# jackvial/tuatara

Hardware: AMD Instinct MI355X
Metric: pages/sec whole-node (1024x768, ~40 crops/page) (higher is better)
Workload: dtype f16x4

## Files before the change

include/tuatara_hip_debug.h:

```cpp
#ifndef TUATARA_HIP_DEBUG_H
#define TUATARA_HIP_DEBUG_H

#include "tuatara_hip.h"

#ifdef __cplusplus
extern "C" {
#endif

int ttr_dbg_conv(ttr_engine* e, const float* in0, int C0, const float* in1, int C1, int relu0, int relu1, int B, int H, int W,
                 int ks, int dil, const float* wgt, const float* bias, int Cout, int act, float* out);

int ttr_dbg_split_gemm(ttr_engine* e, const float* x, int M, int K, const float* w, const float* bias, int N, int np, int act, int out_planes,
                       const float* resid, int cfg, float* out);
int ttr_dbg_conv_pool(ttr_engine* e, const float* in0, int C0, int B, int H, int W, int ks, const float* wgt, const float* bias,
                      int Cout, int act, int pool_relu, float* out_full, float* out_pool);
int ttr_dbg_craft_taps(ttr_engine* e, const uint8_t* canvas, int B, int H, int W, float* heat_out);
int ttr_dbg_craft_tap_count(ttr_engine* e);
int ttr_dbg_craft_tap_info(ttr_engine* e, int i, char* text, size_t cap, int dims[7]);
int ttr_dbg_craft_tap_read(ttr_engine* e, int i, float* out);
void ttr_set_gemm_config(int cfg);
void ttr_set_decoder_mode(int mode);
int ttr_set_tuning(const char* key, int value);
void ttr_last_host_us(ttr_engine* e, float out[8]);
int ttr_dbg_attn_enc(ttr_engine* e, const float* qkv, int N, float* out);
int ttr_dbg_cross_attn(ttr_engine* e, const float* q, const float* kvmem, int N, int R, float* out);
int ttr_dbg_qkv_attn(ttr_engine* e, const float* x, int N, const float* w, const float* b, float* out);
int ttr_dbg_mlp(ttr_engine* e, const float* x, int M, const float* ln_g, const float* ln_b, float eps, const float* w1, const float* b1, const float* w2,
                const float* b2, const float* nln_g, const float* nln_b, float* x_out, float* nln_out, const float* att, const float* wp, const float* bp);
int ttr_dbg_dec_stamps(unsigned long long* out);
int ttr_dbg_dec_stamps_ext(unsigned long long* out, int n);
int ttr_bench_conv(ttr_engine* e, int B, int H, int W, int C0, int C1, int ks, int dil, int Cout, int act, int f32_resid,
                   int iters, float* avg_us);

int ttr_dbg_min_area_rect(const float* xy, int n, float* rect5);
int ttr_dbg_tcp_share(int rank, int world, const char* addr, int port, void* buf, size_t bytes);
int ttr_dbg_component_rect(int area, int x0, int y0, int x1, int y1, const int32_t* rows, int H, int W, float* rect5);
int ttr_dbg_box_geometry(const float* rect5, float ratio, float* adjusted5, int32_t* xywh, float* bbox4);
int ttr_dbg_deskew(const float* rect5, float* quad8, double* coef6, int64_t* fixed6);
int ttr_dbg_orient_quad(const float* rect5, int h, int w, int crop_mode, int turn, float* quad8, int64_t* fixed6);
int ttr_dbg_canvas_geometry(int h, int w, int canvas_size, float mag_ratio, int* H, int* W, float* ratio, int* target_h, int* target_w);


#ifdef __cplusplus
}
#endif
#endif
```

tuatara_amd/csrc/capi_debug.cpp:

```cpp
#include "engine.h"

using namespace ttr;

extern "C" {

int ttr_dbg_conv(ttr_engine* e, const float* in0, int C0, const float* in1, int C1, int relu0, int relu1, int B, int H, int W, int ks, int dil,
                 const float* wgt, const float* bias, int Cout, int act, float* out) {
  TTR_GUARD_BEGIN
  Engine& E = *e->e;
  EngineScope lk(E);
  const size_t M = (size_t)B * H * W;
  const int K = ks * ks * (C0 + C1);
  DevBuf d0, d1, dout;
  Linear L;
  auto up = [&](DevBuf& d, const float* src, size_t nel) {
    d.ensure(nel * E.es);
    if (E.prec == kBF16) {
      std::vector<uint16_t> hbuf(nel);
      for (size_t i = 0; i < nel; ++i) hbuf[i] = f32_to_bf16_rne(src[i]);
      TTR_HIP_CHECK(hipMemcpy(d.p, hbuf.data(), nel * 2, hipMemcpyHostToDevice));
    } else TTR_HIP_CHECK(hipMemcpy(d.p, src, nel * 4, hipMemcpyHostToDevice));
  };
  up(d0, in0, M * C0);
  if (C1) up(d1, in1, M * C1);
// ... 19 lines not shown
  TTR_GUARD_END(-1)
}

int ttr_dbg_split_gemm(ttr_engine* e, const float* x, int M, int K, const float* w, const float* bias, int N, int np, int act, int out_planes,
                       const float* resid, int cfg, float* out) {
  TTR_GUARD_BEGIN
  Engine& E = *e->e;
  EngineScope lk(E);
  if (E.prec != kSplit) throw std::runtime_error("ttr_dbg_split_gemm: f16x4 engines only");
  if ((np != 3 && np != 4) || (out_planes != 0 && out_planes != 2 && out_planes != 3)) throw std::runtime_error("ttr_dbg_split_gemm: np must be 3 or 4, out_planes 0, 2 or 3");
  const int ipl = np == 3 ? 2 : 3;
  DevBuf dx, dxp, dout, dres;
  Linear L;
  dx.ensure((size_t)M * K * 4); TTR_HIP_CHECK(hipMemcpy(dx.p, x, (size_t)M * K * 4, hipMemcpyHostToDevice));
  dxp.ensure((size_t)M * K * 2 * ipl);
  launch_split_planes(dx.as<float>(), K, dxp.p, M, K, 0, E.stream, ipl);
  E.upload_linear(L, w, N, K, bias, cfg == 7 ? (N + 7) / 8 * 8 : N, K, nullptr, false);
  if (!L.ws.p) throw std::runtime_error("ttr_dbg_split_gemm: the layer has no weight planes");
  if (resid) { dres.ensure((size_t)M * N * 4); TTR_HIP_CHECK(hipMemcpy(dres.p, resid, (size_t)M * N * 4, hipMemcpyHostToDevice)); }
  dout.ensure((size_t)M * N * (out_planes ? 2 * out_planes : 4));
  ConvParams p{};
  p.in0 = dxp.p; p.C0 = K; p.B = 1; p.H = 1; p.W = M; p.ks = 1; p.dil = 1;
  if (E.tn.sp_tiled_w) E.tile_planes(L);
  p.wgt = L.ws.p; p.bias = bias ? L.b.as<float>() : nullptr; p.split = np; p.out_scale = L.inv_scale; p.out_planes = out_planes;
  p.wgt_tiled = E.tn.sp_tiled_w ? L.wst.p : nullptr;
  if (out_planes) { p.out = dout.p; p.out_ld = N; } else { p.out_f32 = dout.as<float>(); p.out_f32_ld = N; }
  p.resid = resid ? dres.as<float>() : nullptr; p.resid_ld = N;
  p.Cout = N; p.M = M; p.act = act;
  if (cfg == 7) launch_gemm_skx(p, E.stream);
  else {
    if (const char* err = gemm2_check(p)) throw std::runtime_error(err);
    launch_gemm2(p, cfg, E.stream);
  }
  if (!out_planes) {
    TTR_HIP_CHECK(hipMemcpyAsync(out, dout.p, (size_t)M * N * 4, hipMemcpyDeviceToHost, E.stream));
    TTR_HIP_CHECK(hipStreamSynchronize(E.stream));
    return 0;
  }
  std::vector<uint16_t> h((size_t)M * N * out_planes);
  TTR_HIP_CHECK(hipMemcpyAsync(h.data(), dout.p, h.size() * 2, hipMemcpyDeviceToHost, E.stream));
  TTR_HIP_CHECK(hipStreamSynchronize(E.stream));
  auto f16_to_f32 = [](uint16_t v) -> double {
    const int sgn = v >> 15, ex = (v >> 10) & 31, man = v & 1023;
    double r = ex == 0 ? std::ldexp((double)man, -24) : ex == 31 ? (man ? NAN : INFINITY) : std::ldexp((double)(man | 1024), ex - 25);
    return sgn ? -r : r;
  };
  for (int m = 0; m < M; ++m)
    for (int n = 0; n < N; ++n) {
      const uint16_t* row = h.data() + (size_t)m * out_planes * N;
      double v = f16_to_f32(row[n]), lo = f16_to_f32(row[N + n]);
      if (out_planes == 3) lo += f16_to_f32(row[2 * N + n]);
      out[(size_t)m * N + n] = (float)(v + lo / 2048.0);
    }
  return 0;
  TTR_GUARD_END(-1)
}

int ttr_dbg_mlp(ttr_engine* e, const float* x, int M, const float* ln_g, const float* ln_b, float eps, const float* w1, const float* b1, const float* w2,
                const float* b2, const float* nln_g, const float* nln_b, float* x_out, float* nln_out, const float* att, const float* wp, const float* bp) {
  TTR_GUARD_BEGIN
  Engine& E = *e->e;
  EngineScope lk(E);
  if (E.prec != kBF16) throw std::runtime_error("ttr_dbg_mlp: bf16 engines only");
  const int D = 384, H = 1536;
  DevBuf dx, dout, dg, db, dw1, db1, dw2, db2, dng, dnb, dn;
  auto upf = [&](DevBuf& d, const float* src, size_t n) { d.ensure(n * 4); TTR_HIP_CHECK(hipMemcpy(d.p, src, n * 4, hipMemcpyHostToDevice)); };
  upf(dx, x, (size_t)M * D); upf(dg, ln_g, D); upf(db, ln_b, D); upf(db1, b1, H); upf(db2, b2, D);
  if (nln_out) { upf(dng, nln_g, D); upf(dnb, nln_b, D); dn.ensure((size_t)M * D * 2); }
  std::vector<uint16_t> h((size_t)H * D);
  pack_mlp_w1(w1, h.data());
  dw1.ensure(h.size() * 2); TTR_HIP_CHECK(hipMemcpy(dw1.p, h.data(), h.size() * 2, hipMemcpyHostToDevice));
  pack_mlp_w2(w2, H, h.data());
  dw2.ensure(h.size() * 2); TTR_HIP_CHECK(hipMemcpy(dw2.p, h.data(), h.size() * 2, hipMemcpyHostToDevice));
  dout.ensure((size_t)M * D * 4);
  MlpParams q{};
  q.x = dx.as<float>(); q.x_out = dout.as<float>(); q.M = M; q.ln_g = dg.as<float>(); q.ln_b = db.as<float>(); q.ln_eps = eps;
  q.w1p = dw1.as<bf16>(); q.b1 = db1.as<float>(); q.w2p = dw2.as<bf16>(); q.b2 = db2.as<float>();
  if (nln_out) { q.nln_g = dng.as<float>(); q.nln_b = dnb.as<float>(); q.nln_eps = eps; q.nln_out = dn.as<bf16>(); }
  DevBuf datt, dwp, dbp;
  if (att) {
    std::vector<uint16_t> ha((size_t)M * D), hw((size_t)D * D);
    for (size_t i = 0; i < ha.size(); ++i) ha[i] = f32_to_bf16_rne(att[i]);
    pack_mlp_w2(wp, D, hw.data());
    datt.ensure(ha.size() * 2); TTR_HIP_CHECK(hipMemcpy(datt.p, ha.data(), ha.size() * 2, hipMemcpyHostToDevice));
    dwp.ensure(hw.size() * 2); TTR_HIP_CHECK(hipMemcpy(dwp.p, hw.data(), hw.size() * 2, hipMemcpyHostToDevice));
    upf(dbp, bp, D);
    q.att = datt.as<bf16>(); q.wpp = dwp.as<bf16>(); q.bp = dbp.as<float>();
  }
  launch_mlp_fused(q, E.stream);
  TTR_HIP_CHECK(hipMemcpyAsync(x_out, dout.p, (size_t)M * D * 4, hipMemcpyDeviceToHost, E.stream));
  TTR_HIP_CHECK(hipStreamSynchronize(E.stream));
  if (nln_out) {
    std::vector<uint16_t> hb((size_t)M * D);
    TTR_HIP_CHECK(hipMemcpy(hb.data(), dn.p, hb.size() * 2, hipMemcpyDeviceToHost));
    for (size_t i = 0; i < hb.size(); ++i) { const uint32_t u = (uint32_t)hb[i] << 16; memcpy(&nln_out[i], &u, 4); }
  }
  return 0;
  TTR_GUARD_END(-1)
}

int ttr_dbg_qkv_attn(ttr_engine* e, const float* x, int N, const float* w, const float* b, float* out) {
  TTR_GUARD_BEGIN
  Engine& E = *e->e;
  EngineScope lk(E);
  if (E.prec == kSplit) {
    const size_t nx = (size_t)N * 128 * 384;
// ... 175 lines not shown
    const _Float16* row = h.data() + m * npl * ld;
    float* o = out + m * ld;
    if (npl == 3) for (size_t c = 0; c < ld; ++c) o[c] = (float)row[c] + ((float)row[ld + c] + (float)row[2 * ld + c]) * (1.f / 2048.f);
    else for (size_t c = 0; c < ld; ++c) o[c] = (float)row[c] + (float)row[ld + c] * (1.f / 2048.f);
  }
  return 0;
  TTR_GUARD_END(-1)
}

void ttr_set_gemm_config(int cfg) { set_gemm_config(cfg); }

void ttr_set_decoder_mode(int mode) { g_tuning_default.decoder_mode = mode; }

void ttr_last_host_us(ttr_engine* e, float out[8]) { for (int i = 0; i < 8; ++i) out[i] = e ? e->e->host_us[i] : 0.f; }

int ttr_dbg_dec_stamps_ext(unsigned long long* out, int n) { return g_dec_dbg && n >= 0 && n <= 4096 && hipMemcpy(out, g_dec_dbg, (size_t)n * 8, hipMemcpyDeviceToHost) == hipSuccess ? 0 : -1; }
int ttr_dbg_dec_stamps(unsigned long long* out) { return g_dec_dbg && hipMemcpy(out, g_dec_dbg, 26 * 16 * 8, hipMemcpyDeviceToHost) == hipSuccess ? 0 : -1; }

int ttr_set_tuning(const char* key, int value) {
  const std::string k = key ? key : "";
  if (g_tuning_default.set(k, value)) return 0;
  if (k == "gemm_config") set_gemm_config(value);
  else if (k == "self_refine") set_dec_self_refine(value);
  else if (k == "cross_mfma") set_dec_cross_mfma(value);
  else if (k == "cross_crop") set_dec_cross_crop(value);
  else if (k == "cross_split") set_dec_cross_split(value);
  else if (k == "cross_rows_hsplit") set_dec_cross_rows_hsplit(value);
  else if (k == "mlp_store_nt") set_mlp_store_nt(value);
  else if (k == "mlp_stagger") set_mlp_stagger(value);
  else if (k == "c3s_wgs") set_conv3s_wgs_per_cu(value);
  else if (k == "c3_c32") set_conv3p_c32_tile(value);
  else if (k == "c3_narrow64") set_conv3p_narrow_bn64(value);
  else if (k == "upsample_block") set_upsample_block(value);
  else if (k == "mlp_ablate") set_mlp_ablate(value);
  else if (k == "attn_impl") set_attn_impl(value);
  else if (k == "ws_dbg_flags") set_gemm_ws_dbg_flags(value);
  else if (k == "ws_lean") set_gemm_ws_lean(value);
  else if (k == "store_policy") set_store_policy(value);
  else if (k == "head_persistent") set_conv3p_head_persistent(value);
  else if (k == "up_resident") set_gemm2_up_resident(value);
  else if (k == "up_2d") set_gemm2_up_2d(value);
  else if (k == "c3h_wgs_per_cu") set_conv3h_wgs_per_cu(value);
  else if (k == "g2_x_ring3") set_gemm2_x_ring3(value);
  else if (k == "g2_split_reuse") set_gemm2_split_reuse(value);
  else if (k == "g2_split_cfg") set_gemm2_split_cfg(value);
  else if (k == "g2_split_few") set_gemm2_split_few(value);
  else if (k == "g2_split_dbg") set_gemm2_split_dbg(value);
  else if (k == "g2_split_wreg") set_gemm2_split_wreg(value);
  else if (k == "g2_split_stream") set_gemm2_split_stream(value);
  else if (k == "g2_split_stream4") set_gemm2_split_stream4(value);
  else if (k == "gsp_sched") set_gemm_sp_sched(value);
  else if (k == "gsp_few") set_gemm_sp_few(value);
  else if (k == "gsp_epi") set_gemm_sp_epi(value);
  else if (k == "gsp_ks3") set_gemm_sp_ks3(value);
  else if (k == "gsp_stagger") set_gemm_sp_stagger(value);
  else if (k == "gsp_dbg") set_gemm_sp_dbg(value);
  else if (k == "gsp_stag") set_gemm_sp_stag(value);
  else if (k == "gsp_stagger_groups") set_gemm_sp_stagger_groups(value);
  else if (k == "qkv_attn_dbg") set_qkv_attn_dbg(value);
  else if (k == "qkv_attn4") set_qkv_attn4(value);
  else if (k == "skx_ln_max_rows") set_gemm_skx_ln_max_rows(value);
  else if (k == "c3_xs1_max_cin") set_conv3p_single_stage_max_cin(value);
  else if (k == "c3_force_bn128") set_conv3p_force_bn128(value);
  else if (k == "c3_c64_waves") set_conv3p_c64_waves(value);
  else if (k == "c3_c128_waves") set_conv3p_c128_waves(value);
  else if (k == "c3_narrow_wide") set_conv3p_narrow_wide(value);
  else if (k == "c3_narrow_frac") set_conv3p_narrow_frac(value);
  else if (k == "c3_narrowest_frac") set_conv3p_narrowest_frac(value);
  else if (k == "c3_deep_w") set_conv3p_deep_w(value);
  else if (k == "c3_deep_w64") set_conv3p_deep_w64(value);
  else if (k == "c3_first_persistent") set_conv3p_first_persistent(value);
  else if (k == "sk_max_rows") set_skinny_max_rows(value);
  else if (k == "ws_min_rows") set_gemm_ws_min_rows(value);
  else if (k == "dec_stamps") {
    if (value && !g_dec_dbg) { void* d = nullptr; if (hipMalloc(&d, 4096 * 8) != hipSuccess) return -1; (void)hipMemset(d, 0, 4096 * 8); g_dec_dbg = (unsigned long long*)d; }
    if (!value) g_dec_dbg = nullptr;
    set_gemm_ws_stamps(value == 2 ? g_dec_dbg : nullptr);
    set_conv3p_stamps(value == 4 ? g_dec_dbg : nullptr);
    set_mlp_stamps(value == 3 ? g_dec_dbg : nullptr);
    set_qkv_attn_stamps(value == 5 ? g_dec_dbg : nullptr);
    set_qkv_attn4_stamps(value == 5 ? g_dec_dbg : nullptr);
    set_conv3h_stamps(value == 6 ? g_dec_dbg : nullptr);
  }
  else return -1;
  return 0;
}

int ttr_engine_set_tuning(ttr_engine* e, const char* key, int value) {
  TTR_GUARD_BEGIN
  if (!e) return -1;
  const std::string k = key ? key : "";
  {
    std::lock_guard<std::mutex> lk(e->e->mu);
    if (e->e->tn.set(k, value)) return 0;
  }
  return ttr_set_tuning(key, value);
  TTR_GUARD_END(-1)
}

int ttr_bench_conv(ttr_engine* e, int B, int H, int W, int C0, int C1, int ks, int dil, int Cout, int act, int f32_resid, int iters, float* avg_us) {
  TTR_GUARD_BEGIN
  Engine& E = *e->e;
  EngineScope lk(E);
  const size_t M = (size_t)B * H * W;
  const int K = ks * ks * (C0 + C1);
  DevBuf d0, d1, dw, db, dout, dres;
// ... 103 lines not shown
```

tuatara_amd/csrc/common.h:

```cpp
#pragma once
#include <hip/hip_runtime.h>

#include <atomic>
#include <mutex>
#include <stdint.h>

namespace ttr {

typedef __bf16 bf16;
typedef __attribute__((ext_vector_type(8))) __bf16 bf16x8;
typedef __attribute__((ext_vector_type(4))) float f32x4;

enum Precision { kBF16 = 0, kF32 = 1, kSplit = 2 };
enum Act { kActNone = 0, kActRelu = 1, kActGelu = 2 };

struct ClassMask {
  uint32_t blocked[3];
  __host__ __device__ __forceinline__ bool allows(int c) const { return (unsigned)c >= 96u || !((blocked[c >> 5] >> (c & 31)) & 1u); }
  __host__ __device__ __forceinline__ bool restricts() const { return (blocked[0] | blocked[1] | blocked[2]) != 0u; }
};

typedef uint4 RowMask;
struct RowClassMask {
  uint32_t b0, b1, b2;
  __device__ __forceinline__ bool allows(int c) const { return (unsigned)c >= 96u || !(((c < 32 ? b0 : (c < 64 ? b1 : b2)) >> (c & 31)) & 1u); }
};
__device__ __forceinline__ RowClassMask row_class_mask(const ClassMask& cm, const RowMask* __restrict__ rows, int row) {
  RowClassMask m{cm.blocked[0], cm.blocked[1], cm.blocked[2]};
  if (rows) {
    const RowMask r = rows[__builtin_amdgcn_readfirstlane(row)];
    m.b0 = r.x; m.b1 = r.y; m.b2 = r.z;
  }
  return m;
}

struct ConvParams {
  const void* in0; int C0;
  const void* in1; int C1;
  int relu0, relu1;
  int B, H, W;
  int ks, dil;
  const void* wgt;
  int x_tiled, out_tiled;
  const void* wgt_tiled;
  const float* bias;
  void* out; int out_ld;
  float* out_f32; int out_f32_ld;
  void* out_relu;
  void* out_pool; int pool_relu;
  const float* resid; int resid_ld; int resid_mod;
  int Cout, M, act;
  const void* pre_wgt; const float* pre_bias;
  float pre_scale;
  unsigned pre_range_tag;
  const float* ln_in; int ln_ld; const float* ln_gamma; const float* ln_beta; float ln_eps;
  int* tok; int tok_ld, tok_col; const float* tok_logits; int tok_logits_ld, tok_C; const float* tok_emb; const float* tok_pos; int tok_max;
  ClassMask tok_mask;
  const RowMask* tok_row_masks;
  unsigned long long* dbg;
  int store_policy;
  int dbg_flags;
  const int* skip; int skip_n;
  int* done_count; int tok_eos;
  const void* gelu_lut;
  int split; float out_scale; int out_planes;
  int out_full_cols;
  const void* tail_w6; const void* tail_w8; const float* tail_b6; const float* tail_b8; float tail_s6, tail_s8; float* tail_heat;
  const float* up_z; int up_ld;
  int up_2d;
  unsigned* range_flag; unsigned range_tag;
  int cu_stagger, cu_stagger_groups;
  unsigned* tile_ctr;
};

__device__ __forceinline__ float gelu_exact(float x) { return 0.5f * x * (1.0f + erff(x * 0.70710678118654752440f)); }

__device__ __forceinline__ float gelu_fast(float x) {
  const float z = fabsf(x) * 0.70710678118654752440f;
  const float t = __frcp_rn(1.0f + 0.3275911f * z);
  const float poly = t * (0.254829592f + t * (-0.284496736f + t * (1.421413741f + t * (-1.453152027f + t * 1.061405429f))));
  const float e = 1.0f - poly * __expf(-z * z);
  return 0.5f * x * (1.0f + copysignf(e, x));
}

__device__ __forceinline__ float gelu_lut(float x, const float2* lut) {
  const float u = fmaf(__builtin_amdgcn_fmed3f(x, -8.0f, 7.984375f), 64.0f, 512.0f);
  const float2 t = lut[(int)u];
  return x * fmaf(__builtin_amdgcn_fractf(u), t.y, t.x);
}

__device__ __forceinline__ float gelu_hermite(float x, const float2* lut) {
  const float u = fmaf(__builtin_amdgcn_fmed3f(x, -8.0f, 7.96875f), 32.0f, 256.0f);
  const float4 c = reinterpret_cast<const float4*>(lut)[(int)u];
  const float t = __builtin_amdgcn_fractf(u);
  return x * fmaf(fmaf(fmaf(c.w, t, c.z), t, c.y), t, c.x);
}

__device__ __forceinline__ void gelu_hermite8(float (&v)[8], const float2* lut) {
  float u[8];
  float4 c[8];
#pragma unroll
  for (int e = 0; e < 8; ++e) {
    u[e] = fmaf(__builtin_amdgcn_fmed3f(v[e], -8.0f, 7.96875f), 32.0f, 256.0f);
    c[e] = reinterpret_cast<const float4*>(lut)[(int)u[e]];
  }
#pragma unroll
  for (int e = 0; e < 8; ++e) {
    const float t = __builtin_amdgcn_fractf(u[e]);
    v[e] = v[e] * fmaf(fmaf(fmaf(c[e].w, t, c[e].z), t, c[e].y), t, c[e].x);
  }
}

__device__ __forceinline__ void gelu_lut8_lds(float (&v)[8], unsigned lut_lds) {
  float u[8];
  float2 t[8];
#pragma unroll
  for (int e = 0; e < 8; ++e) {
    u[e] = fmaf(__builtin_amdgcn_fmed3f(v[e], -8.0f, 7.984375f), 64.0f, 512.0f);
    const unsigned a = lut_lds + ((unsigned)(int)u[e] << 3);
    asm volatile("ds_read_b64 %0, %1" : "=v"(t[e]) : "v"(a));
  }
  asm volatile("s_waitcnt lgkmcnt(0)"
               : "+v"(t[0]), "+v"(t[1]), "+v"(t[2]), "+v"(t[3]), "+v"(t[4]), "+v"(t[5]), "+v"(t[6]), "+v"(t[7]));
#pragma unroll
  for (int e = 0; e < 8; ++e) v[e] = v[e] * fmaf(__builtin_amdgcn_fractf(u[e]), t[e].y, t[e].x);
// ... 45 lines not shown
```

tuatara_amd/csrc/engine.h:

```cpp
#pragma once
#include <algorithm>
#include <cmath>
#include <cstdio>
#include <cstring>
#include <fstream>
#include <iostream>
#include <iterator>
#include <map>
#include <memory>
#include <mutex>
#include <chrono>
#include <dlfcn.h>
#include <arpa/inet.h>
#include <netdb.h>
#include <netinet/in.h>
#include <netinet/tcp.h>
#include <sys/socket.h>
#include <unistd.h>
#include <rccl/rccl.h>

#include <atomic>
#include <functional>
#include <condition_variable>
#include <thread>
#include <stdexcept>
#include <string>
#include <vector>

#include "../../include/tuatara_hip_debug.h"
#include "common.h"
#include "geometry.h"
#include "host_util.h"
#include "kernels.h"

namespace ttr {


extern thread_local std::string g_last_error;
extern unsigned long long* g_dec_dbg;
struct Tuning {
  int dbg_bf16_out = 0;
  int qkv_attn = 1;
  int qkv_attn_min = 160;
  int mlp_proj = 1;
  int mlp_min_rows = 49152;
  int dec_mlp_fused = 1;
  int dec_mlp_min_rows = 16384;
  int mlp_fused = 1;
  int tok_fuse = 1;
  int ln_fuse = 1;
  int fuse_first = 1;
  int qkv_attn_split = 1;
  int skinny_split = 1;
  int skinny_max_rows = 2048;
  int skx_ln_fuse = 1;
  int embed_fold = 1;
  int argmax_fold = 1;
  int sp_tiled_x = 1;
  int sp_tiled_w = 1;
  int ar_host_check = 10;
  int enc_chunk = 0;
  int enc_ln_pairs = 1;
  int dec_planes = 1;
  int qkv_kv_pairs = 1;
  int enc_fc2_pairs = 1;
  int craft_products = 3;
  int gpu_calipers = 1;
  int up_commute = 1;
  int head_tail = 1;
  int first_fused = 1;
  int head_packed = 1;
  int detector_only = 0;
  int bench_grid_boxes = 0;
  int split_planes = 1;
  int split_conv3p = 1;
  int split_gemm = 1;
  int craft_group = 16;
  int ar_tail_step = 12;
  int ar_crop_exit = 1;
  int ar_early_exit = 1;
  int decoder_mode = 1;
  int sp_hidden16 = 0;
  int craft_lanes = 1;
  int recog_overlap = 1;
  int images_batch = 32;
  int range_guard = 1;
  bool set(const std::string& k, int value) {
    if (k == "decoder_mode") decoder_mode = value;
    else if (k == "enc_chunk") enc_chunk = value;
    else if (k == "range_guard") range_guard = value;
    else if (k == "recog_overlap") recog_overlap = value;
    else if (k == "craft_lanes") craft_lanes = value == 2 ? 2 : 1;
    else if (k == "sp_hidden16") sp_hidden16 = value;
    else if (k == "images_batch") images_batch = value < 1 ? 1 : (value > 256 ? 256 : value);
    else if (k == "up_commute") up_commute = value;
    else if (k == "gpu_calipers") gpu_calipers = value;
    else if (k == "skinny_split") skinny_split = value;
    else if (k == "skinny_max_rows") skinny_max_rows = value;
    else if (k == "ar_host_check") ar_host_check = value;
    else if (k == "sp_tiled_w") sp_tiled_w = value;
    else if (k == "sp_tiled_x") sp_tiled_x = value;
    else if (k == "argmax_fold") argmax_fold = value;
    else if (k == "embed_fold") embed_fold = value;
    else if (k == "skx_ln_fuse") skx_ln_fuse = value;
    else if (k == "qkv_attn_split") qkv_attn_split = value;
    else if (k == "fuse_first") fuse_first = value;
    else if (k == "ln_fuse") ln_fuse = value;
    else if (k == "tok_fuse") tok_fuse = value;
    else if (k == "ar_early_exit") ar_early_exit = value;
    else if (k == "ar_crop_exit") ar_crop_exit = value;
    else if (k == "ar_tail_step") ar_tail_step = value;
    else if (k == "split_gemm") split_gemm = value;
    else if (k == "bench_grid_boxes") bench_grid_boxes = value;
    else if (k == "detector_only") detector_only = value;
    else if (k == "craft_products") craft_products = value == 4 ? 4 : 3;
    else if (k == "head_packed") head_packed = value;
    else if (k == "first_fused") first_fused = value;
    else if (k == "head_tail") head_tail = value;
    else if (k == "enc_ln_pairs") enc_ln_pairs = value;
    else if (k == "enc_fc2_pairs") enc_fc2_pairs = value;
    else if (k == "qkv_kv_pairs") qkv_kv_pairs = value;
    else if (k == "dec_planes") dec_planes = value;
    else if (k == "split_conv3p") split_conv3p = value;
    else if (k == "split_planes") split_planes = value;
    else if (k == "craft_group") craft_group = value < 1 ? 1 : (value > 32 ? 32 : value);
    else if (k == "mlp_fused") mlp_fused = value;
    else if (k == "mlp_min_rows") mlp_min_rows = value;
    else if (k == "dec_mlp_fused") dec_mlp_fused = value;
    else if (k == "dec_mlp_min_rows") dec_mlp_min_rows = value;
    else if (k == "mlp_proj") mlp_proj = value;
    else if (k == "qkv_attn") qkv_attn = value;
    else if (k == "qkv_attn_min") qkv_attn_min = value;
    else if (k == "dbg_bf16_out") dbg_bf16_out = value;
    else return false;
    return true;
  }
};
extern Tuning g_tuning_default;

struct Roctx {
  int (*push)(const char*) = nullptr; int (*pop)() = nullptr;
  Roctx() {
// ... 311 lines not shown

  static int qkv_tile_row(int n) {
    const int h = n / 192, c = n % 192, wn = c / 96, t = (c % 96) / 32, dd = c % 32;
    return 384 * t + 64 * h + 32 * wn + dd;
  }

  void load_head_tail(WeightFile& wf);
  void load_parseq(const std::string& dir);

  bool verbose = false;
  enum { kRangeDet0 = 0, kRangeDet1 = 1, kRangeRec0 = 2, kRangeRec1 = 3, kRangeStage = 4, kRangeWords = 8 };
  DevBuf range_word;
  PinnedBuf h_range;
  std::vector<std::string> range_names;
  std::map<std::string, unsigned> range_ids;
  std::string range_scope;
  unsigned* range_flag_ptr(int w = kRangeStage) { return prec == kSplit && tn.range_guard ? range_word.as<unsigned>() + w : nullptr; }
  void range_use(int w) { range_ctx().flag = range_flag_ptr(w); }
  void range_tag(const std::string& layer);
  void range_fetch(int w);
  void range_verify(int w, const char* where);
  Comm* comm = nullptr;
  DevBuf gath_dev[2];
  PinnedBuf h_gath[2];
  struct Gathered { int world = 0, pages = 0; std::vector<int32_t> counts, ids; std::vector<float> prob, conf; } last_gathered;
  void allgather_host(const void* mine, size_t bytes, void* all);
  Engine(const std::string& dir, const ttr_config& c);
  ~Engine();

  DevBuf& ws(size_t idx, size_t bytes, bool zero_new = false);

  void conv(const char* name, const void* in0, int C0, const void* in1, int C1, int relu0, int B, int H, int W, void* out, int act,
            float* out_f32 = nullptr, void* out_relu = nullptr, void* out_pool = nullptr, int pool_relu = 0);

  void craft_forward(const uint8_t* d_canvas, int B, int H, int W, float* d_heat);


  void upconv_commuted(const char* name, const void* y_lo, int C0, const void* skip, int C1, int B, int H, int W, float* z, void* out);
  const uint8_t* sconv_canvas = nullptr;
  void sconv(const char* name, const void* in0, int C0, const void* in1, int C1, int B, int H, int W, void* out, int act,
             void* out_relu = nullptr, void* out_pool = nullptr, int pool_relu = 0, int out_planes = -1, int out_ld = 0, bool packed = false, float* tail_heat = nullptr);
  void craft_forward_split(const uint8_t* d_canvas, int B, int H, int W, float* d_heat);
  enum { kTapF32 = 0, kTapPacked = 1, kTapPairs = 2, kTapTriples = 3, kTapU8 = 4 };
  struct CraftTap {
    std::string layer, role, kind;
    const void* p; int B, H, W, C, ld, form;
  };
  bool craft_tap_on = false;
  std::vector<CraftTap> craft_taps;
  void tap(const char* layer, const char* role, const void* p, int B, int H, int W, int C, int ld, int form, const char* kind = "") {
    if (craft_tap_on && p) craft_taps.push_back(CraftTap{layer, role, kind, p, B, H, W, C, ld, form});
  }

  void sgemm(const Linear& L, const void* in_planes, int M, void* out, int out_ld, int act, int out_planes,
             float* out_f32 = nullptr, int out_f32_ld = 0, const float* resid = nullptr, int resid_ld = 0, int np = 4, int resid_mod = 0, int out_full_cols = 0,
             const char* kind = nullptr, int x_tiled = 0, int out_tiled = 0);
  void ln_gemm(const float* x, const std::string& ln_name, float eps, void* scratch, const Linear& L, int M, void* out, int out_ld, int act,
               float* out_f32 = nullptr, int out_f32_ld = 0);
  void gemm(const Linear& L, const void* in, int M, void* out, int out_ld, int act, float* out_f32 = nullptr, int out_f32_ld = 0,
            const float* resid = nullptr, int resid_ld = 0, int resid_mod = 0);
  const int* cur_skip = nullptr; int cur_skip_n = 0;
  DevBuf ar_done;
  PinnedBuf h_ar_done;
  bool streaming_recog = false;
  size_t kvcache_zeroed = 0;
  void ln(const float* x, const std::string& name, float eps, void* out, int M);

  void decoder_tail_split(const void* sa, int N, int R, const float* resid_pos, int resid_mod, float* tgt, void* pa, void* pb, void* p1536, float* q384,
                          void* t384, const void* kvmem, float* logits_out, int logits_ld, const int* done_tok = nullptr, int done_col = 0);

  void decoder_tail(const void* sa, int N, int R, const float* resid_pos, int resid_mod, float* tgt, void* t384, void* t384b, void* t1536,
                    const void* kvmem, float* logits_out, int logits_ld, const int* done_tok = nullptr, int done_col = 0);

  void parseq_forward(const uint8_t* d_crops, int N, float* d_logits, float* d_ar, int* d_ids, float* d_prob, float* d_conf, const RowMask* row_masks = nullptr);
  struct RecOut { int* ids; float* prob; float* conf; };
  static constexpr int kRecWords = 26 + 26 + 1;
  static constexpr int kLogitWords = 26 * 95;
  RecOut rec_out(int rows) { return rec_block(ids_dev, rows); }
  static RecOut rec_block(DevBuf& d, int rows) {
    d.ensure((size_t)std::max(rows, 1) * kRecWords * 4);
    int* b = d.as<int>();
    return RecOut{b, reinterpret_cast<float*>(b + (size_t)rows * 26), reinterpret_cast<float*>(b + (size_t)rows * 52)};
  }
  struct RecRows { const int32_t* ids; const float* prob; const float* conf; };
  static RecRows rec_rows(const void* block, int rows) {
    const int32_t* b = static_cast<const int32_t*>(block);
    return RecRows{b, reinterpret_cast<const float*>(b + (size_t)rows * 26), reinterpret_cast<const float*>(b + (size_t)rows * 52)};
  }
  int orient_k() const { return cfg.orient == TTR_ORIENT_QUARTER ? 4 : cfg.orient == TTR_ORIENT_FLIP ? 2 : 1; }

  struct PageBoxes { std::vector<RRect> det; };

  void ccl_launch(const float* d_heat, int p0, int pages, int total, int g, int H2, int W2, int lane = 0);
  void ccl_collect(int p0, int pages, int g, int H2, int W2, std::vector<std::vector<RRect>>& det);
  void parallel_pages(int pages, const std::function<void(int)>& f) { host_pool->run(pages, f); }

  struct Page { const uint8_t* data = nullptr; int h = 0, w = 0, stride = 0; CanvasGeom g{}; };
  struct PageBatch {
    const uint8_t* d_pages = nullptr; int n = 0, h = 0, w = 0;
    bool mixed = false;
    std::vector<Page> pages;
    int H = 0, W = 0, H2 = 0, W2 = 0;
    std::vector<std::vector<RRect>> boxes;
    std::vector<int> rects, page_of;
    std::vector<int64_t> coef;
    std::vector<int64_t> twin;
    int N = 0, slot = 0, group = 16;
    int det_groups = -1;
    bool live = false, enqueued = false;
// ... 94 lines not shown
```

tuatara_amd/csrc/engine_parseq.cpp:

```cpp
#include "engine.h"

namespace ttr {

unsigned long long* g_dec_dbg = nullptr;

void Engine::sgemm(const Linear& L, const void* in_planes, int M, void* out, int out_ld, int act, int out_planes,
           float* out_f32, int out_f32_ld, const float* resid, int resid_ld, int np, int resid_mod, int out_full_cols,
           const char* kind, int x_tiled, int out_tiled) {
  if (!L.ws.p) throw std::runtime_error("split GEMM: the layer has no weight planes");
  range_tag("parseq." + range_scope + (kind ? kind : "linear"));
  ConvParams p{};
  p.out_full_cols = out_full_cols;
  p.in0 = in_planes; p.C0 = L.k; p.B = 1; p.H = 1; p.W = M; p.ks = 1; p.dil = 1;
  p.wgt = L.ws.p; p.bias = L.b.as<float>(); p.split = np; p.out_scale = L.inv_scale; p.out_planes = out_planes == 1 ? 3 : out_planes;
  p.wgt_tiled = tn.sp_tiled_w ? L.wst.p : nullptr;
  p.x_tiled = x_tiled; p.out_tiled = out_tiled;
  p.store_policy = out_tiled == 2 && tn.sp_hidden16 == 2 ? 1 : 0;
  p.out = out; p.out_ld = out_ld; p.out_f32 = out_f32; p.out_f32_ld = out_f32_ld; p.resid = resid; p.resid_ld = resid_ld; p.resid_mod = resid_mod;
  p.Cout = L.cout_valid ? L.cout_valid : L.cout; p.M = M; p.act = act;
  p.skip = cur_skip; p.skip_n = cur_skip_n;
  const bool skinny = tn.skinny_split && np == 4 && M <= tn.skinny_max_rows && !x_tiled && !out_tiled && gemm_skx_eligible(p);
  if (!skinny) { if (const char* e = gemm2_check(p)) throw std::runtime_error(e); }
  if (skinny) {
    timed(kind ? kind : "split linear (triples, skinny)", 2.0 * M * p.Cout * L.k, 2.0 * M * p.Cout * L.k * np, [&] { launch_gemm_skx(p, stream); });
    return;
  }
  timed(kind ? kind : (np == 3 ? "split linear (pairs)" : "split linear (triples)"), 2.0 * M * L.cout * L.k, 2.0 * M * L.cout * L.k * np, [&] { launch_gemm2(p, 0, stream); });
}

void Engine::ln_gemm(const float* x, const std::string& ln_name, float eps, void* scratch, const Linear& L, int M, void* out, int out_ld, int act,
             float* out_f32, int out_f32_ld) {
  if (tn.ln_fuse && prec == kBF16 && L.k == 384 && M <= skinny_max_rows()) {
    ConvParams p{};
    p.ln_in = x; p.ln_ld = 384; p.ln_gamma = pqf.at(ln_name + ".weight").as<float>(); p.ln_beta = pqf.at(ln_name + ".bias").as<float>(); p.ln_eps = eps;
    p.C0 = L.k; p.B = 1; p.H = 1; p.W = M; p.ks = 1; p.dil = 1;
    p.wgt = L.w.p; p.bias = L.b.as<float>();
    p.out = out; p.out_ld = out_ld; p.out_f32 = out_f32; p.out_f32_ld = out_f32_ld;
    p.Cout = L.cout; p.M = M; p.act = act;
    p.skip = cur_skip; p.skip_n = cur_skip_n;
    igemm(p, 2.0 * M * L.cout * L.k);
    return;
  }
  ln(x, ln_name, eps, scratch, M);
  gemm(L, scratch, M, out, out_ld, act, out_f32, out_f32_ld);
}

void Engine::gemm(const Linear& L, const void* in, int M, void* out, int out_ld, int act, float* out_f32, int out_f32_ld,
          const float* resid, int resid_ld, int resid_mod) {
  ConvParams p{};
  p.in0 = in; p.C0 = L.k; p.B = 1; p.H = 1; p.W = M; p.ks = 1; p.dil = 1;
  p.wgt = L.w.p; p.bias = L.b.as<float>();
  p.out = out; p.out_ld = out_ld; p.out_f32 = out_f32; p.out_f32_ld = out_f32_ld;
  p.resid = resid; p.resid_ld = resid_ld; p.resid_mod = resid_mod;
  p.Cout = L.cout_valid ? L.cout_valid : L.cout; p.M = M; p.act = act;
  p.skip = cur_skip; p.skip_n = cur_skip_n;
  igemm(p, 2.0 * M * p.Cout * L.k);
}

void Engine::ln(const float* x, const std::string& name, float eps, void* out, int M) {
  launch_layernorm(prec, x, 384, pqf.at(name + ".weight").as<float>(), pqf.at(name + ".bias").as<float>(), eps, out, 384, M, 384, stream, cur_skip, cur_skip_n);
}

void Engine::decoder_tail_split(const void* sa, int N, int R, const float* resid_pos, int resid_mod, float* tgt, void* pa, void* pb, void* p1536, float* q384,
                        void* t384, const void* kvmem, float* logits_out, int logits_ld, const int* done_tok, int done_col) {
  const int rows = N * R;
  const std::string d = "decoder.layers.0.";
  auto lnp = [&](const std::string& nm, void* out) {
    range_tag("parseq." + nm);
    launch_layernorm_planes(tgt, 384, pqf.at(nm + ".weight").as<float>(), pqf.at(nm + ".bias").as<float>(), 1e-5f, out, rows, stream, 3, cur_skip, cur_skip_n);
  };
  auto ln_lin = [&](const std::string& nm, const Linear& L, void* out, int out_ld, int act, int out_planes, float* out_f32, int out_f32_ld, const char* kind) {
    range_tag("parseq." + range_scope + kind);
    ConvParams p{};
    p.ln_in = tgt; p.ln_ld = 384; p.ln_gamma = pqf.at(nm + ".weight").as<float>(); p.ln_beta = pqf.at(nm + ".bias").as<float>(); p.ln_eps = 1e-5f;
// ... 26 lines not shown
void Engine::decoder_tail(const void* sa, int N, int R, const float* resid_pos, int resid_mod, float* tgt, void* t384, void* t384b, void* t1536,
                  const void* kvmem, float* logits_out, int logits_ld, const int* done_tok, int done_col) {
  const int rows = N * R;
  const std::string d = "decoder.layers.0.";
  gemm(pq.at("self_out"), sa, rows, nullptr, 0, kActNone, tgt, 384, resid_pos, 384, resid_mod);
  ln_gemm(tgt, d + "norm1", 1e-5f, t384, pq.at("cross_q"), rows, t384b, 384, kActNone);
  launch_dec_cross_attn(prec, t384b, kvmem, t384, N, R, stream, cur_skip, cur_skip_n, done_tok, done_col);
  const int dec_panels = (rows + 127) / 128, dec_cus = device_cu_count(256), dec_rounds = (dec_panels + dec_cus - 1) / dec_cus;
  const bool dec_fill = tn.dec_mlp_fused == 2 || dec_panels * 100 >= 65 * dec_rounds * dec_cus;
  if (R > 1 && prec == kBF16 && gemm_config() >= 0 && tn.dec_mlp_fused && rows >= tn.dec_mlp_min_rows && dec_fill) {
    MlpParams q{};
    q.x = tgt; q.x_out = tgt; q.M = rows;
    q.ln_g = pqf.at(d + "norm2.weight").as<float>(); q.ln_b = pqf.at(d + "norm2.bias").as<float>(); q.ln_eps = 1e-5f;
    q.w1p = dec_ffn1_packed.as<bf16>(); q.b1 = pq.at("ffn1").b.as<float>();
    q.w2p = dec_ffn2_packed.as<bf16>(); q.b2 = pq.at("ffn2").b.as<float>();
    q.nln_g = pqf.at("decoder.norm.weight").as<float>(); q.nln_b = pqf.at("decoder.norm.bias").as<float>(); q.nln_eps = 1e-5f; q.nln_out = (bf16*)t384b;
    q.att = (const bf16*)t384; q.wpp = dec_co_packed.as<bf16>(); q.bp = pq.at("cross_out").b.as<float>();
    timed("mlp_fused (refinement block)", 2.0 * rows * 384 * 1536 * 2 + 2.0 * rows * 384 * 384, 2.0 * rows * 384 * 1536 * 2 + 2.0 * rows * 384 * 384, [&] { launch_mlp_fused(q, stream); });
    gemm(pq.at("head"), t384b, rows, nullptr, 0, kActNone, logits_out, logits_ld);
    return;
  }
  gemm(pq.at("cross_out"), t384, rows, nullptr, 0, kActNone, tgt, 384, tgt, 384, 0);
  ln_gemm(tgt, d + "norm2", 1e-5f, t384, pq.at("ffn1"), rows, t1536, 1536, kActGelu);
  gemm(pq.at("ffn2"), t1536, rows, nullptr, 0, kActNone, tgt, 384, tgt, 384, 0);
  ln_gemm(tgt, "decoder.norm", 1e-5f, t384, pq.at("head"), rows, nullptr, 0, kActNone, logits_out, logits_ld);
}

void Engine::parseq_forward(const uint8_t* d_crops, int N, float* d_logits, float* d_ar, int* d_ids, float* d_prob, float* d_conf, const RowMask* row_masks) {
  if (N <= 0) return;
  constexpr int kMaxCrops = 4096;
  if (N > kMaxCrops) {
    const int groups = (N + kMaxCrops - 1) / kMaxCrops, per = (N + groups - 1) / groups;
    for (int g0 = 0; g0 < N; g0 += per) {
      const int n = std::min(per, N - g0);
      parseq_forward(d_crops + (size_t)g0 * 32 * 128 * 3, n, d_logits + (size_t)g0 * 26 * 95, d_ar ? d_ar + (size_t)g0 * 26 * 95 : nullptr, d_ids + (size_t)g0 * 26,
                     d_prob + (size_t)g0 * 26, d_conf + g0, row_masks ? row_masks + g0 : nullptr);
    }
    return;
  }
  if ((charset.restricts() || row_masks) && prec == kBF16) throw std::runtime_error("parseq_forward: a character set needs an f16x4 or f32 engine (the bf16 engine's kernels take no class mask)");
  prof_stage = 1;
  const int M = N * 128, E = 384;
  const int patch_ld = pq.at("patch").k;
  range_tag("parseq.encoder.patch_embed");
  void* patches = (pq_ws[0].ensure((size_t)M * patch_ld * es), pq_ws[0].p);
  float* x = (float*)(pq_ws[1].ensure((size_t)M * E * 4), pq_ws[1].p);
  void* t384 = (pq_ws[2].ensure((size_t)std::max(M, N * 26) * E * es), pq_ws[2].p);
  void* tbig = (pq_ws[3].ensure((size_t)M * 1536 * es), pq_ws[3].p);
  void* att = (pq_ws[4].ensure((size_t)std::max(M, N * 26) * E * es), pq_ws[4].p);
  launch_patchify(prec, d_crops, patches, N, patch_ld, stream);
  gemm(pq.at("patch"), patches, M, nullptr, 0, kActNone, x, E, pqf.at("encoder.pos_embed").as<float>(), E, 128);
  const bool enc_split = prec == kSplit && tn.split_gemm && tn.split_planes;
  if (enc_split) {
    int CHS = std::max(1, std::min(N, (int)((((size_t)1 << 31) - 1) / ((size_t)128 * 1536 * 6))));
    if (tn.enc_chunk > 0) CHS = std::min(CHS, tn.enc_chunk);
    if (N > CHS) { const int groups = (N + CHS - 1) / CHS; CHS = (N + groups - 1) / groups; }
    void* lnp = (pq_ws[11].ensure((size_t)M * E * 6), pq_ws[11].p);
    void* bigp = (pq_ws[12].ensure((size_t)std::min(N, CHS) * 128 * 1536 * 6), pq_ws[12].p);
    void* attp = (pq_ws[13].ensure((size_t)std::min(N, CHS) * 128 * E * 6), pq_ws[13].p);
    auto lnp_at = [&](int c0) { return (char*)lnp + (size_t)c0 * 128 * E * 6; };
    const int lnpl = tn.enc_ln_pairs ? 2 : 3;
    const int xt = tn.sp_tiled_x && tn.qkv_attn_split && lnpl == 2 && tn.enc_fc2_pairs && std::min(CHS, N) * 128 > tn.skinny_max_rows ? 1 : 0;
    for (int c0 = 0; c0 < N; c0 += CHS) {
      const int nc = std::min(CHS, N - c0), Mc = nc * 128;
      float* xc = x + (size_t)c0 * 128 * E;
      for (int l = 0; l < 12; ++l) {
        const std::string p = "encoder.blocks." + std::to_string(l) + ".";
        range_scope = p;
        range_tag("parseq." + p + "norm1");
        launch_layernorm_planes(xc, E, pqf.at(p + "norm1.weight").as<float>(), pqf.at(p + "norm1.bias").as<float>(), 1e-6f, lnp_at(c0), Mc, stream, lnpl, nullptr, 0, xt);
        if (tn.qkv_attn_split && lnpl == 2) {
          const Linear& L = pq.at(p + "qkv_hm");
          range_tag("parseq." + p + "attn (qkv + attention)");
          const double qa = 2.0 * Mc * 3 * E * E, aa = 2.0 * 2 * nc * 6 * 128.0 * 128 * 64;
          timed("enc.qkv+attention: gemm_sp_kernel<128,192,NP=3,EPI=1>", qa + aa, qa * 3 + aa * 3.5,
                [&] { launch_qkv_attn_split(lnp_at(c0), L.ws.p, L.b.as<float>(), L.inv_scale, attp, nc, stream, tn.sp_tiled_w ? L.wst.p : nullptr, xt, xt); });
        } else {
        sgemm(pq.at(p + "qkv"), lnp_at(c0), Mc, bigp, 3 * E, kActNone, 1, nullptr, 0, nullptr, 0, lnpl + 1, 0, tn.qkv_kv_pairs ? E : 0, "enc.qkv");
        range_tag("parseq." + p + "attn.qkv"), launch_attn_enc_split(bigp, attp, nc, stream);
        }
        sgemm(pq.at(p + "proj"), attp, Mc, nullptr, 0, kActNone, 0, xc, E, xc, E, 4, 0, 0, "enc.proj", xt, 0);
        range_tag("parseq." + p + "norm2");
        launch_layernorm_planes(xc, E, pqf.at(p + "norm2.weight").as<float>(), pqf.at(p + "norm2.bias").as<float>(), 1e-6f, lnp_at(c0), Mc, stream, lnpl, nullptr, 0, xt);
        const int hpl = tn.enc_fc2_pairs ? 2 : 3;
        const int hx = xt && tn.sp_hidden16 && hpl == 2 ? 2 : xt;
        sgemm(pq.at(p + "fc1"), lnp_at(c0), Mc, bigp, 4 * E, kActGelu, hpl, nullptr, 0, nullptr, 0, lnpl + 1, 0, 0, "enc.fc1 + GELU", xt, hx);
        sgemm(pq.at(p + "fc2"), bigp, Mc, nullptr, 0, kActNone, 0, xc, E, xc, E, hpl + 1, 0, 0, "enc.fc2", hx, 0);
      }
      range_scope.clear();
      range_tag("parseq.encoder.norm");
      launch_layernorm_planes(xc, E, pqf.at("encoder.norm.weight").as<float>(), pqf.at("encoder.norm.bias").as<float>(), 1e-6f, lnp_at(c0), Mc, stream);
    }
  }
  const bool mlp_fused = prec == kBF16 && gemm_config() >= 0 && (tn.mlp_fused == 2 || (tn.mlp_fused == 1 && M >= tn.mlp_min_rows));
  const int CH = (tn.enc_chunk > 0 && !mlp_fused) ? tn.enc_chunk : N;
  for (int c0 = 0; c0 < N && !enc_split; c0 += CH) {
    const int nc = std::min(CH, N - c0), Mc = nc * 128;
    float* xc = x + (size_t)c0 * 128 * E;
    if (mlp_fused) ln(xc, "encoder.blocks.0.norm1", 1e-6f, t384, Mc);
    for (int l = 0; l < 12; ++l) {
      std::string p = "encoder.blocks." + std::to_string(l) + ".";
      if (!mlp_fused) ln(xc, p + "norm1", 1e-6f, t384, Mc);
      if (prec == kBF16 && gemm_config() >= 0 && (tn.qkv_attn == 2 || (tn.qkv_attn == 1 && nc >= tn.qkv_attn_min)) && (size_t)Mc * E * 2 < ((size_t)1 << 31)) {
        const Linear& L = pq.at(p + "qkv");
        timed("qkv_attn_kernel", 2.0 * Mc * E * 3 * E, 2.0 * Mc * E * 3 * E, [&] { launch_qkv_attn((const bf16*)t384, L.w.as<bf16>(), L.b.as<float>(), (bf16*)att, nc, stream); });
      } else {
        gemm(pq.at(p + "qkv"), t384, Mc, tbig, 3 * E, kActNone);
        launch_attn_enc(prec, tbig, att, nc, stream);
      }
      const bool proj_in = mlp_fused && tn.mlp_proj;
      if (!proj_in) gemm(pq.at(p + "proj"), att, Mc, nullptr, 0, kActNone, xc, E, xc, E, 0);
      if (mlp_fused) {
        const std::string nx = l < 11 ? "encoder.blocks." + std::to_string(l + 1) + ".norm1" : std::string("encoder.norm");
        MlpParams q{};
        q.x = xc; q.x_out = xc; q.M = Mc;
        q.ln_g = pqf.at(p + "norm2.weight").as<float>(); q.ln_b = pqf.at(p + "norm2.bias").as<float>(); q.ln_eps = 1e-6f;
        q.w1p = fc1_packed[l].as<bf16>(); q.b1 = pq.at(p + "fc1").b.as<float>();
        q.w2p = fc2_packed[l].as<bf16>(); q.b2 = pq.at(p + "fc2").b.as<float>();
        q.nln_g = pqf.at(nx + ".weight").as<float>(); q.nln_b = pqf.at(nx + ".bias").as<float>(); q.nln_eps = 1e-6f; q.nln_out = (bf16*)t384;
        if (proj_in) { q.att = (const bf16*)att; q.wpp = proj_packed[l].as<bf16>(); q.bp = pq.at(p + "proj").b.as<float>(); }
        q.no_x_store = l == 11;
        const double mf = 2.0 * Mc * E * 4 * E * 2 + (proj_in ? 2.0 * Mc * E * E : 0.0);
        timed("mlp_fused_kernel", mf, mf, [&] { launch_mlp_fused(q, stream); });
        continue;
      }
      ln(xc, p + "norm2", 1e-6f, t384, Mc);
      gemm(pq.at(p + "fc1"), t384, Mc, tbig, 4 * E, kActGelu);
      gemm(pq.at(p + "fc2"), tbig, Mc, nullptr, 0, kActNone, xc, E, xc, E, 0);
    }
  }
  if (!mlp_fused && !enc_split) ln(x, "encoder.norm", 1e-6f, t384, M);
  void* kvmem = (pq_ws[5].ensure((size_t)M * 768 * es), pq_ws[5].p);
  if (enc_split) {
    const int rows_max = (int)((((size_t)1 << 31) - 1) / ((size_t)E * 6));
    for (int r0 = 0; r0 < M; r0 += rows_max) {
      const int rr = std::min(rows_max, M - r0);
      sgemm(pq.at("cross_kv"), (char*)pq_ws[11].p + (size_t)r0 * E * 6, rr, (char*)kvmem + (size_t)r0 * 768 * 4, 768, kActNone, 0);
    }
  } else
  gemm(pq.at("cross_kv"), t384, M, kvmem, 768, kActNone);

  range_scope = "decoder.";
  struct ScopeReset { std::string& s; ~ScopeReset() { s.clear(); } } scope_reset{range_scope};
  void* kvcache = (pq_ws[6].ensure((size_t)N * 26 * 768 * es), pq_ws[6].p);
// ... 146 lines not shown
```

tuatara_amd/csrc/gemm2.hip:

```cpp
#include <algorithm>
#include <cmath>
#include <mutex>
#include <type_traits>
#include <vector>

#include "common.h"
#include "kernels.h"
#include "split.h"

namespace ttr {

#ifndef TTR_ST_OUT
#define TTR_ST_OUT
__device__ __forceinline__ void st_out(bf16* dst, bf16x8 v, int policy) {
  if (policy == 1 || policy == 2) __builtin_nontemporal_store(v, reinterpret_cast<bf16x8*>(dst));
  else *reinterpret_cast<bf16x8*>(dst) = v;
}
#endif

typedef __attribute__((address_space(3))) void* lds_ptr;

__device__ __forceinline__ __amdgpu_buffer_rsrc_t make_rsrc(const void* base, unsigned bytes) {
  return __builtin_amdgcn_make_buffer_rsrc(const_cast<void*>(base), 0, (int)bytes, 0x00020000);
}
// ... 567 lines not shown
  if ((size_t)p.M * p.C0 * es_in >= lim || (size_t)p.M * p.C1 * es_in >= lim || (size_t)p.Cout * K * 2 >= lim) return "gemm2: tensor too large for 32-bit buffer offsets";
  if (p.M != p.B * p.H * p.W || p.M <= 0 || p.Cout <= 0) return "gemm2: bad shape";
  if (p.split && !(p.out_scale > 0.f)) return "gemm2: split mode needs out_scale";
  if (p.up_z && (!p.split || p.ks != 1 || p.C1 || (p.H & 1) || (p.W & 1) || p.up_ld % 4 || p.up_ld < p.Cout || ((uintptr_t)p.up_z & 15) || p.out_pool || p.resid))
    return "gemm2: the half-resolution addend (up_z) is the split mode's, on a single-source 1x1 layer over even H and W";
  return nullptr;
}

static int g_up_2d = 0;
void set_gemm2_up_2d(int v) { g_up_2d = v; }
static int g_up_resident = 1;
void set_gemm2_up_resident(int v) { g_up_resident = v; }
void launch_gemm2(const ConvParams& p_in, int cfg, hipStream_t s) {
  if (const char* e = gemm2_check(p_in)) throw std::runtime_error(e);
  if (g_up_resident && cfg == 0 && conv1u_eligible(p_in)) return launch_conv1u(p_in, s);
  ConvParams p = p_in;
  const int Ctot = p.C0 + p.C1;
  p.gelu_lut = p.act == kActGelu ? (p.split ? gelu_hermite_lut_for_current_device() : gelu_lut_for_current_device()) : nullptr;
  if (cfg == 0 && p.split && g_split_cfg) cfg = g_split_cfg;
  if (cfg == 0 && p.split && p.Cout > 64) {
    const int64_t t2 = (int64_t)((p.M + 255) / 256) * ((p.Cout + 127) / 128);
    cfg = t2 >= 2 * num_cus() ? 2 : 3;
    if (cfg == 2 && p.Cout >= 1024 && p.ks == 1 && p.M >= 65536) cfg = 6;
  }
  if (cfg == 0) {
    if (p.Cout <= 64) cfg = 5;
    else {
      cfg = 3;
      if (p.Cout % 256 == 0) {
        const int64_t tiles = (int64_t)((p.M + 255) / 256) * (p.Cout / 256);
        const double eff = (double)tiles / (double)(((tiles + 255) / 256) * 256);
        if (tiles >= 1024 || (tiles <= 256 && eff >= 0.74) || eff >= 0.85) cfg = 1;
      }
      if (cfg == 3 && g_x_ring3 && p.act != kActGelu && (int64_t)((p.M + 255) / 256) * ((p.Cout + 127) / 128) >= 512) cfg = 2;
    }
  }
  const bool deep = g_x_ring3 && p.act != kActGelu;
  if (p.split) p.dbg_flags = g_split_dbg;
  if (p.up_z && cfg == 1) cfg = 2;
  {
    const int bm = (cfg == 1 || cfg == 2 || cfg == 4) ? 256 : 128;
    p.up_2d = (g_up_2d && p.up_z && !p.out_pool && p.W % 16 == 0 && p.H % (bm / 16) == 0 && p.M % bm == 0 && p.M == p.B * p.H * p.W) ? 1 : 0;
  }
  if (p.split && cfg == 1) p.gelu_lut = nullptr;
  if (p.split == 4 && (cfg == 2 || cfg == 3 || cfg == 6) && g_split_stream && g_split_stream4 && gemm_sp_eligible(p)) return launch_gemm_sp(p, cfg, s);
  if (p.split == 3 && (cfg == 2 || cfg == 3 || cfg == 6) && g_split_stream && gemm_sp_eligible(p)) {
    int sc = cfg;
    if (g_split_stream == 1 || (p.Cout < 512 && Ctot >= 1024)) sc = 3;
    return launch_gemm_sp(p, sc, s);
  }
  if (p.split == 3 && p.ks == 3 && (cfg == 2 || cfg == 3) && g_split_stream && gemm_sp_ks3_eligible(p))
    return launch_gemm_sp_ks3(p, cfg, s);
  if (p.x_tiled || p.out_tiled) throw std::runtime_error("gemm2: tiled planes are gemm_sp.hip's (this shape did not qualify for it)");
  if (p.split && cfg == 3 && g_split_few && (int64_t)((p.M + 127) / 128) * ((p.Cout + 127) / 128) <= num_cus()) cfg = 5;
  if (p.split) {
    const bool ru = g_split_reuse != 0 || p.split == 3;
    if (p.split == 3) {
      switch (cfg) {
        case 1: return launch_g2<256, 256, 2, 4, 1, 3, 3>(p, s);
        case 2: return g_split_wreg ? launch_g2<256, 128, 4, 2, 1, 3, 3, 3>(p, s) : launch_g2<256, 128, 4, 2, 1, 3, 3>(p, s);
        case 3: return launch_g2<128, 128, 2, 2, 2, 3, 3>(p, s);
        case 4: return launch_g2<256, 64, 4, 1, 1, 3, 3>(p, s);
        case 5: return launch_g2<128, 64, 2, 2, 2, 3, 3>(p, s);
        case 6: return g_split_wreg ? launch_g2<128, 256, 2, 4, 1, 3, 3, 3>(p, s) : launch_g2<128, 256, 2, 4, 1, 3, 3>(p, s);
        default: throw std::runtime_error("gemm2: unknown configuration");
      }
    }
    switch (cfg) {
      case 1: return ru ? launch_g2<256, 256, 2, 4, 1, 3, 4>(p, s) : launch_g2<256, 256, 2, 4, 1, 2, 4>(p, s);
      case 2: return ru ? (g_split_wreg ? launch_g2<256, 128, 4, 2, 1, 3, 4, 3>(p, s) : launch_g2<256, 128, 4, 2, 1, 3, 4>(p, s)) : launch_g2<256, 128, 4, 2, 1, 2, 4>(p, s);
      case 3: return ru ? launch_g2<128, 128, 2, 2, 2, 3, 4>(p, s) : launch_g2<128, 128, 2, 2, 2, 2, 4>(p, s);
      case 4: return ru ? launch_g2<256, 64, 4, 1, 1, 3, 4>(p, s) : launch_g2<256, 64, 4, 1, 2, 2, 4>(p, s);
      case 5: return ru ? launch_g2<128, 64, 2, 2, 2, 3, 4>(p, s) : launch_g2<128, 64, 2, 2, 2, 2, 4>(p, s);
      case 6: return ru ? (g_split_wreg ? launch_g2<128, 256, 2, 4, 1, 3, 4, 3>(p, s) : launch_g2<128, 256, 2, 4, 1, 3, 4>(p, s)) : launch_g2<128, 256, 2, 4, 1, 2, 4>(p, s);
      default: throw std::runtime_error("gemm2: unknown configuration");
    }
  }
  switch (cfg) {
    case 1: return deep ? launch_g2<256, 256, 2, 4, 1, 3>(p, s) : launch_g2<256, 256, 2, 4, 1, 2>(p, s);
    case 2: return deep ? launch_g2<256, 128, 4, 2, 1, 3>(p, s) : launch_g2<256, 128, 4, 2, 1, 2>(p, s);
    case 3: return deep ? launch_g2<128, 128, 2, 2, 2, 3>(p, s) : launch_g2<128, 128, 2, 2, 2, 2>(p, s);
    case 4: return launch_g2<256, 64, 4, 1, 2, 2>(p, s);
    case 5: return launch_g2<128, 64, 2, 2, 2, 2>(p, s);
    case 6: return deep ? launch_g2<128, 256, 2, 4, 1, 3>(p, s) : launch_g2<128, 256, 2, 4, 1, 2>(p, s);
    default: throw std::runtime_error("gemm2: unknown configuration");
  }
}

template <typename T>
__global__ void fill_random_kernel(T* p, size_t n, unsigned seed, float scale) {
  for (size_t i = (size_t)blockIdx.x * blockDim.x + threadIdx.x; i < n; i += (size_t)gridDim.x * blockDim.x) {
    unsigned h = (unsigned)i * 2654435761u ^ (unsigned)(i >> 32) ^ (seed * 0x9E3779B9u);
    h ^= h >> 16; h *= 0x7feb352du; h ^= h >> 15; h *= 0x846ca68bu; h ^= h >> 16;
    p[i] = (T)(((float)(h >> 8) * (1.0f / 8388608.0f) - 1.0f) * scale);
  }
}

void launch_fill_random(Precision prec, void* p, size_t n, unsigned seed, float scale, hipStream_t s) {
  if (n == 0) return;
  const int grid = (int)std::min<size_t>((n + 255) / 256, 65536);
  if (prec == kBF16) hipLaunchKernelGGL(fill_random_kernel<bf16>, dim3(grid), dim3(256), 0, s, (bf16*)p, n, seed, scale);
  else hipLaunchKernelGGL(fill_random_kernel<float>, dim3(grid), dim3(256), 0, s, (float*)p, n, seed, scale);
}

}
```

tuatara_amd/csrc/gemm_sp.hip:

```cpp
#include <algorithm>
#include <stdexcept>
#include <type_traits>

#include "common.h"
#include "kernels.h"
#include "split.h"

namespace ttr {

typedef __attribute__((address_space(3))) void* lds_ptr;

static __device__ __forceinline__ __amdgpu_buffer_rsrc_t sp_rsrc(const void* base, unsigned bytes) {
  return __builtin_amdgcn_make_buffer_rsrc(const_cast<void*>(base), 0, (int)bytes, 0x00020000);
}

static __device__ __forceinline__ void sp_store_f32x8(float* o, const float (&v)[8]) {
  __builtin_nontemporal_store(f32x4{v[0], v[1], v[2], v[3]}, reinterpret_cast<f32x4*>(o));
  __builtin_nontemporal_store(f32x4{v[4], v[5], v[6], v[7]}, reinterpret_cast<f32x4*>(o + 4));
}

template <int BM, int BN, int WM, int WN, int XST, int WST>
struct SpCfg {
  static constexpr int NW = WM * WN, NT = NW * 64;
  static constexpr int TM = BM / WM, TN = BN / WN;
  static constexpr int MI = TM / 16, NJ = TN / 16;
  static constexpr int XPW = BM / 8 / NW, WPW = BN / 8 / NW;
  static constexpr int XBYTES = BM * 128, WBYTES = BN * 128;
  static constexpr int LDS = XST * XBYTES + WST * WBYTES;
  static_assert((XST == 2 || XST == 3) && (WST == 2 || WST == 3) && !(XST == 2 && WST == 3), "ring depths: (3, 3), (3, 2) or (2, 2)");
  static_assert((BM / 8) % NW == 0 && (BN / 8) % NW == 0 && TN % 32 == 0 && TM % 16 == 0, "tile shape");
};

template <int BM, int BN, int WM, int WN, int XST, int WST, int MINB, bool SCHED, int NP, int EPI = 0, int EM = 0, bool KS3 = false, int DBG = 0, bool STAG = false>
__global__ __launch_bounds__(WM * WN * 64, MINB) void gemm_sp_kernel(ConvParams p) {
  using C = SpCfg<BM, BN, WM, WN, XST, WST>;
  static_assert(NP == 3 || (NP == 4 && XST == 3 && WST == 2), "pairs, or triples on rings 3 + 2");
  static_assert(EPI == 0 || (EPI == 1 && BM == 128 && BN == 192 && WM == 4 && WN == 2 && NP == 3), "attention epilogue: 128 x 192 tiles on 4 x 2 waves, activation pairs");
  constexpr int PLX = NP == 3 ? 2 : 3;
  if (p.skip && __builtin_nontemporal_load(p.skip) >= p.skip_n) return;
  extern __shared__ __attribute__((aligned(1024))) unsigned char smem[];
  const int tid = threadIdx.x, lane = tid & 63;
  const int wave = __builtin_amdgcn_readfirstlane(tid >> 6);
  const int wm = wave / WN, wn = wave % WN;

  static_assert(EM == 0 || EPI == 0, "fixed epilogue cases are the plain epilogue's");
  static_assert(!KS3 || (NP == 3 && EPI == 0), "3x3 taps: the pairs loop");
  static_assert(!STAG || (NP == 3 && WM * WN == 8 && SCHED), "staggered halves: the pairs loop on eight waves");
  float2* const glut = reinterpret_cast<float2*>(smem + C::LDS);
  if (EM == 1 || EM == 3 || (EM == 0 && p.act == kActGelu && p.gelu_lut)) {
    for (int i = tid; i < 512; i += C::NT) reinterpret_cast<uint4*>(glut)[i] = reinterpret_cast<const uint4*>(p.gelu_lut)[i];
  }

  const int tilesM = (p.M + BM - 1) / BM, tilesN = (p.Cout + BN - 1) / BN;
  const int T = tilesM * tilesN;
  const int xcd = blockIdx.x & 7, J = gridDim.x >> 3;
  int xcd_first, xcd_count;
  {
    const int q = T >> 3, r = T & 7;
    xcd_first = xcd < r ? xcd * (q + 1) : r * (q + 1) + (xcd - r) * q;
    xcd_count = q + (xcd < r ? 1 : 0);
  }
  int idx = blockIdx.x >> 3;
  if (idx >= xcd_count) return;
  if (p.cu_stagger > 0) {
    const unsigned long long wait = (unsigned long long)((blockIdx.x >> 3) % p.cu_stagger_groups) * (unsigned)p.cu_stagger / (unsigned)p.cu_stagger_groups;
    const unsigned long long t0 = __builtin_amdgcn_s_memrealtime();
    while (__builtin_amdgcn_s_memrealtime() - t0 < wait) __builtin_amdgcn_s_sleep(32);
  }

  const int K = p.C0, nkt = K >> 6, nk0 = KS3 ? 9 * nkt : nkt;
  const int Kw = KS3 ? 9 * K : K;
  const __amdgpu_buffer_rsrc_t rsx = sp_rsrc(p.in0, (unsigned)((size_t)p.M * K * 2 * PLX));
  const bool wtiled = p.wgt_tiled != nullptr;
  const __amdgpu_buffer_rsrc_t rsw = sp_rsrc(wtiled ? p.wgt_tiled : p.wgt, (unsigned)((size_t)((p.Cout + 31) / 32 * 32) * Kw * 6));
  const unsigned x_plstep = p.x_tiled == 2 ? (unsigned)(K >> 5) * 1024u : p.x_tiled ? (unsigned)(K >> 6) * 1024u : (unsigned)K * 2u;
  const unsigned x_kstep = p.x_tiled == 2 ? 2048u : p.x_tiled ? 1024u : 128u;
  const unsigned w_pl1 = wtiled ? (unsigned)(2 * (K >> 6)) * 1024u : (unsigned)Kw * 4u, w_kstep = wtiled ? 1024u : 128u;
  constexpr unsigned OOB = 0x80000000u;

  unsigned char* const xring = smem;
  unsigned char* const wring = smem + XST * C::XBYTES;

  auto tile_offsets = [&](int li, unsigned (&xo)[C::XPW], unsigned (&wo)[C::WPW]) {
    const bool live = li < xcd_count;
    const int tile = xcd_first + li, tm = tile / tilesN, m0 = tm * BM, n0 = (tile - tm * tilesN) * BN;
#pragma unroll
    for (int i = 0; i < C::XPW; ++i) {
      const int row = (i * C::NW + wave) * 8 + (lane >> 3);
      const int g = (lane & 7) ^ ((row >> 1) & 7);
      const int m = m0 + row;
      if (p.x_tiled == 2) xo[i] = (live && m < p.M) ? ((unsigned)(m >> 4) * (unsigned)(PLX * (K >> 5)) + (unsigned)(g >> 2)) * 1024u + (unsigned)(((g & 3) * 16 + (m & 15)) * 16) : OOB;
      else if (p.x_tiled) xo[i] = (live && m < p.M) ? (unsigned)(m >> 3) * (unsigned)(PLX * (K >> 6)) * 1024u + (unsigned)((m & 7) * 128 + g * 16) : OOB;
      else xo[i] = (live && m < p.M) ? ((unsigned)m * (unsigned)(PLX * K) + g * 8) * 2u : OOB;
    }
#pragma unroll
    for (int j = 0; j < C::WPW; ++j) {
      const int row = (j * C::NW + wave) * 8 + (lane >> 3);
      const int g = (lane & 7) ^ ((row >> 1) & 7);
      const int q16 = row & 15;
      const int nl = (row & ~31) + (q16 >> 2) * 8 + ((row >> 4) & 1) * 4 + (q16 & 3);
      const int n = n0 + nl;
      if (wtiled) wo[j] = (live && n < p.Cout) ? (unsigned)((n0 + (row & ~7)) >> 3) * (unsigned)(3 * (K >> 6)) * 1024u + (unsigned)((row & 7) * 128 + g * 16) : OOB;
      else wo[j] = (live && n < p.Cout) ? ((unsigned)n * (unsigned)(3 * Kw) + g * 8) * 2u : OOB;
    }
  };

  unsigned xvo[C::XPW], wvo[C::WPW], xdl[C::XPW], wdl[C::WPW];
  int xs_k = 0, xs_pl = 0, xs_slot = 0;
  int ws_k = 0, ws_pl = 0, ws_slot = 0;
  unsigned xcen[KS3 ? C::XPW : 1];
  int xyq[KS3 ? C::XPW : 1];
  int xs_tap = 0, xs_li = idx;
  auto x_set_tile = [&](int li) {
    const bool live = li < xcd_count;
    const int tile = xcd_first + li, tm = tile / tilesN, m0 = tm * BM;
#pragma unroll
    for (int i = 0; i < C::XPW; ++i) {
      const int row = (i * C::NW + wave) * 8 + (lane >> 3);
      const int g = (lane & 7) ^ ((row >> 1) & 7);
      const int m = m0 + row;
      const int mm = m < p.M ? m : 0;
      const int xq = mm % p.W, yq = (mm / p.W) % p.H;
      xyq[KS3 ? i : 0] = (yq << 16) | xq;
      xcen[KS3 ? i : 0] = (live && m < p.M) ? ((unsigned)m * (unsigned)(PLX * K) + g * 8) * 2u : OOB;
    }
  };
  auto x_set_tap = [&](int tap) {
    const int ty = tap / 3, dy = (ty - 1) * p.dil, dx = (tap - 3 * ty - 1) * p.dil;
    const unsigned shift = (unsigned)((dy * p.W + dx) * (PLX * K * 2));
#pragma unroll
    for (int i = 0; i < C::XPW; ++i) {
      const int y = (xyq[KS3 ? i : 0] >> 16) + dy, x = (xyq[KS3 ? i : 0] & 0xffff) + dx;
      const bool ok = xcen[KS3 ? i : 0] != OOB && (unsigned)y < (unsigned)p.H && (unsigned)x < (unsigned)p.W;
      xvo[i] = ok ? xcen[KS3 ? i : 0] + shift : OOB;
    }
  };
  auto issue_x = [&]() {
    const unsigned soff = (unsigned)xs_pl * x_plstep + (unsigned)xs_k * x_kstep;
    unsigned char* sb = xring + xs_slot * C::XBYTES + wave * 1024;
#pragma unroll
    for (int i = 0; i < C::XPW; ++i) {
      const unsigned vo = (DBG & 4) ? OOB : (DBG & 8) ? xvo[i] - (xvo[i] != OOB ? xvo[i] / (1u << 20) * (1u << 20) : 0u) : xvo[i];
      if constexpr (!(DBG & 1)) __builtin_amdgcn_raw_ptr_buffer_load_lds(rsx, (lds_ptr)(sb + i * C::NW * 1024), 16, vo, soff, 0, 0);
    }
    xs_slot = xs_slot == XST - 1 ? 0 : xs_slot + 1;
    const bool lastpl = xs_pl == PLX - 1;
    const int k1 = xs_k + (lastpl ? 1 : 0);
    xs_pl = lastpl ? 0 : xs_pl + 1;
    if constexpr (KS3) {
      const bool tapwrap = k1 == nkt;
      xs_k = tapwrap ? 0 : k1;
      if (tapwrap) {
        xs_tap = xs_tap == 8 ? 0 : xs_tap + 1;
        if (xs_tap == 0) { xs_li += J; x_set_tile(xs_li); }
        x_set_tap(xs_tap);
      }
    } else {
    const bool wrap = k1 == nk0;
    xs_k = wrap ? 0 : k1;
    const unsigned mask = wrap ? 0xFFFFFFFFu : 0u;
#pragma unroll
    for (int i = 0; i < C::XPW; ++i) xvo[i] += xdl[i] & mask;
    }
  };
  auto issue_w = [&]() {
    const unsigned soff = (ws_pl ? w_pl1 : 0u) + (unsigned)ws_k * w_kstep;
    unsigned char* sb = wring + ws_slot * C::WBYTES + wave * 1024;
#pragma unroll
    for (int j = 0; j < C::WPW; ++j) {
      const unsigned vo = (DBG & 4) ? OOB : wvo[j];
      if constexpr (!(DBG & 1)) __builtin_amdgcn_raw_ptr_buffer_load_lds(rsw, (lds_ptr)(sb + j * C::NW * 1024), 16, vo, soff, 0, 0);
    }
    ws_slot = ws_slot == WST - 1 ? 0 : ws_slot + 1;
    const int k1 = ws_k + ws_pl;
    ws_pl ^= 1;
    const bool wrap = k1 == nk0;
    ws_k = wrap ? 0 : k1;
    const unsigned mask = wrap ? 0xFFFFFFFFu : 0u;
#pragma unroll
    for (int j = 0; j < C::WPW; ++j) wvo[j] += wdl[j] & mask;
  };
#define TTR_SP_NEXT_DELTAS(LI)                                                   \
  {                                                                              \
    unsigned xa_[C::XPW], wa_[C::WPW], xb_[C::XPW], wb_[C::WPW];                 \
    tile_offsets((LI), xa_, wa_);                                                \
    tile_offsets((LI) + J, xb_, wb_);                                            \
    _Pragma("unroll") for (int i = 0; i < C::XPW; ++i) xdl[i] = xb_[i] - xa_[i]; \
    _Pragma("unroll") for (int j = 0; j < C::WPW; ++j) wdl[j] = wb_[j] - wa_[j]; \
  }

  const int frag_lane = (lane & 15) * 128 + ((((lane >> 4)) ^ ((lane >> 1) & 7)) << 4);
  const int xfo[2] = {wm * C::TM * 128 + frag_lane, wm * C::TM * 128 + (frag_lane ^ 64)};
  const int wfo[2] = {wn * C::TN * 128 + frag_lane, wn * C::TN * 128 + (frag_lane ^ 64)};
  const int fg = lane >> 4, fr = lane & 15;
  int xr = 0, wr = 0;
  f16x8 fx0[2][C::MI], fx1[2][C::MI], fw0[2][C::NJ], fw1[2][C::NJ];
  bool dbg_first = true;
  auto read_x = [&](f16x8 (&f)[2][C::MI]) {
    if constexpr ((DBG & 2) != 0) { if (!dbg_first) { asm volatile("" : "+v"(f[0][0]), "+v"(f[1][0])); return; } }
    const unsigned char* b = xring + xr * C::XBYTES;
#pragma unroll
    for (int kk = 0; kk < 2; ++kk)
#pragma unroll
      for (int i = 0; i < C::MI; ++i) f[kk][i] = *reinterpret_cast<const f16x8*>(b + xfo[kk] + i * 2048);
    xr = xr == XST - 1 ? 0 : xr + 1;
  };
  auto read_w = [&](f16x8 (&f)[2][C::NJ]) {
    if constexpr ((DBG & 2) != 0) { if (!dbg_first) { asm volatile("" : "+v"(f[0][0]), "+v"(f[1][0])); return; } }
    const unsigned char* b = wring + wr * C::WBYTES;
#pragma unroll
    for (int kk = 0; kk < 2; ++kk)
#pragma unroll
      for (int j = 0; j < C::NJ; ++j) f[kk][j] = *reinterpret_cast<const f16x8*>(b + wfo[kk] + j * 2048);
    wr = wr == WST - 1 ? 0 : wr + 1;
  };

  tile_offsets(idx, xvo, wvo);
  TTR_SP_NEXT_DELTAS(idx)
  if constexpr (KS3) { x_set_tile(idx); x_set_tap(0); }
  constexpr int XW = C::XPW + C::WPW;
  constexpr int PH0 = WST == 3 ? XW : C::XPW;
  constexpr int PH1 = XST == 2 ? XW : 63;
  constexpr int PH2 = WST == 3 ? XW + C::WPW : C::WPW;
  constexpr int T0 = 2 * C::XPW, T1 = 2 * C::XPW + C::WPW, T2 = C::XPW + 2 * C::WPW, T3 = XW;
  issue_x(); issue_w();
  if constexpr (NP == 4) {
    issue_w();
    issue_x();
    issue_x();
    asm volatile("s_waitcnt vmcnt(%0)" ::"n"(C::WPW + 2 * C::XPW) : "memory");
  } else if constexpr (XST == 3 && WST == 3) {
    issue_x(); issue_w();
    issue_w();
    issue_x();
    asm volatile("s_waitcnt vmcnt(%0)" ::"n"(2 * XW) : "memory");
  } else if constexpr (XST == 3) {
    issue_x();
    issue_w();
    issue_x();
    asm volatile("s_waitcnt vmcnt(%0)" ::"n"(XW + C::XPW) : "memory");
  } else {
    issue_w();
    issue_x();
    asm volatile("s_waitcnt vmcnt(%0)" ::"n"(XW) : "memory");
  }
  __builtin_amdgcn_s_barrier();
  asm volatile("" ::: "memory");
  read_x(fx0); read_w(fw0);
  if constexpr ((DBG & 2) != 0) { read_x(fx1); read_w(fw1); dbg_first = false; }

  int stamp_tile = 0;
#define TTR_SP_STAMP(ph) do { if (EPI == 1 && p.dbg && blockIdx.x == 0 && tid == 0 && stamp_tile < 24) p.dbg[stamp_tile * 16 + (ph)] = __builtin_readcyclecounter(); } while (0)
  while (true) {
    TTR_SP_STAMP(0);
    if constexpr (EPI == 1) { if (p.dbg && blockIdx.x == 0 && tid == 0 && stamp_tile < 24) p.dbg[stamp_tile * 16 + 11] = __builtin_amdgcn_s_memrealtime(); }
    f32x4 acc[C::NJ][C::MI];
#pragma unroll
    for (int j = 0; j < C::NJ; ++j)
#pragma unroll
      for (int i = 0; i < C::MI; ++i) acc[j][i] = f32x4{0.f, 0.f, 0.f, 0.f};
    const int ctile = xcd_first + idx;
    const int m0c = (ctile / tilesN) * BM, n0c = (ctile % tilesN) * BN;

    auto mfmas = [&](const f16x8 (&fw)[2][C::NJ], const f16x8 (&fx)[2][C::MI]) {
#pragma unroll
      for (int kk = 0; kk < 2; ++kk)
#pragma unroll
        for (int i = 0; i < C::MI; ++i)
#pragma unroll
          for (int j = 0; j < C::NJ; ++j) acc[j][i] = __builtin_amdgcn_mfma_f32_16x16x32_f16(fw[kk][j], fx[kk][i], acc[j][i], 0, 0, 0);
    };
    auto interleave = [&](auto reads_c, auto loads_c) {
      constexpr int READS = decltype(reads_c)::value, LOADS = decltype(loads_c)::value;
#define TTR_SP_GROUP(G)                                                                      \
      __builtin_amdgcn_sched_group_barrier(0x008, 1, 0);                                     \
      __builtin_amdgcn_sched_group_barrier(0x100, READS > 8 ? 2 : 1, 0);                     \
      if constexpr (G < LOADS) __builtin_amdgcn_sched_group_barrier(0x020, 1, 0);
      TTR_SP_GROUP(0) TTR_SP_GROUP(1) TTR_SP_GROUP(2) TTR_SP_GROUP(3) TTR_SP_GROUP(4) TTR_SP_GROUP(5) TTR_SP_GROUP(6) TTR_SP_GROUP(7)
#undef TTR_SP_GROUP
    };
    auto scale_w0 = [&]() {
      const f16 sc = (f16)(1.f / 2048.f);
      const f16x8 scv = {sc, sc, sc, sc, sc, sc, sc, sc};
#pragma unroll
      for (int kk = 0; kk < 2; ++kk)
#pragma unroll
        for (int j = 0; j < C::NJ; ++j) fw1[kk][j] = fw0[kk][j] * scv;
    };
    if constexpr (NP == 4) {
      auto phase_head = [&](auto allow_c) {
        __builtin_amdgcn_sched_barrier(0);
        asm volatile("s_waitcnt vmcnt(%0) lgkmcnt(0)" ::"n"(decltype(allow_c)::value) : "memory");
        __builtin_amdgcn_s_barrier();
        asm volatile("" ::: "memory");
        __builtin_amdgcn_sched_barrier(0);
      };
      auto k_step = [&](f16x8 (&a)[2][C::MI], f16x8 (&b)[2][C::MI]) {
        phase_head(std::integral_constant<int, T0>{});
        issue_x(); issue_w();
        read_w(fw1);
        mfmas(fw0, a);
        if constexpr (SCHED) interleave(std::integral_constant<int, 2 * C::NJ>{}, std::integral_constant<int, XW>{});
        phase_head(std::integral_constant<int, T1>{});
        issue_w();
        read_x(b);
        mfmas(fw1, a);
        if constexpr (SCHED) interleave(std::integral_constant<int, 2 * C::MI>{}, std::integral_constant<int, C::WPW>{});
        __builtin_amdgcn_sched_barrier(0);
        scale_w0();
        phase_head(std::integral_constant<int, T2>{});
        issue_x();
        read_x(a);
        mfmas(fw1, b);
        if constexpr (SCHED) interleave(std::integral_constant<int, 2 * C::MI>{}, std::integral_constant<int, C::XPW>{});
        phase_head(std::integral_constant<int, T3>{});
// ... 41 lines not shown
        read_x(fx1);
        mfmas_kk(fw1, fx0, 0);
        interleave(std::integral_constant<int, 2 * C::MI>{}, std::integral_constant<int, C::WPW>{});
        __builtin_amdgcn_sched_barrier(0);
        scale_w0_kk(0);
        if (!late) { mfmas_kk(fw1, fx0, 1); __builtin_amdgcn_sched_barrier(0); scale_w0_kk(1); }
        head(std::integral_constant<int, PH2>{});
        if (late) { mfmas_kk(fw1, fx0, 1); __builtin_amdgcn_sched_barrier(0); scale_w0_kk(1); }
        __builtin_amdgcn_sched_barrier(0);
        issue_x();
        read_x(fx0); read_w(fw0);
        mfmas_kk(fw1, fx1, 0);
        interleave(std::integral_constant<int, 2 * C::MI + 2 * C::NJ>{}, std::integral_constant<int, C::XPW>{});
        __builtin_amdgcn_sched_barrier(0);
        if (!late) mfmas_kk(fw1, fx1, 1);
      }
      __builtin_amdgcn_sched_barrier(0);
      if (late) mfmas_kk(fw1, fx1, 1);
    } else {
    for (int k0 = 0; k0 < nk0; ++k0) {
      __builtin_amdgcn_sched_barrier(0);
      asm volatile("s_waitcnt vmcnt(%0) lgkmcnt(0)" ::"n"(PH0) : "memory");
      __builtin_amdgcn_s_barrier();
      asm volatile("" ::: "memory");
      __builtin_amdgcn_sched_barrier(0);
      issue_x(); issue_w();
      read_w(fw1);
      mfmas(fw0, fx0);
      if constexpr (SCHED) interleave(std::integral_constant<int, 2 * C::NJ>{}, std::integral_constant<int, XW>{});
      __builtin_amdgcn_sched_barrier(0);
      asm volatile("s_waitcnt vmcnt(%0) lgkmcnt(0)" ::"n"(PH1) : "memory");
      __builtin_amdgcn_s_barrier();
      asm volatile("" ::: "memory");
      __builtin_amdgcn_sched_barrier(0);
      issue_w();
      read_x(fx1);
      mfmas(fw1, fx0);
      if constexpr (SCHED) interleave(std::integral_constant<int, 2 * C::MI>{}, std::integral_constant<int, C::WPW>{});
      __builtin_amdgcn_sched_barrier(0);
      scale_w0();
      __builtin_amdgcn_sched_barrier(0);
      asm volatile("s_waitcnt vmcnt(%0) lgkmcnt(0)" ::"n"(PH2) : "memory");
      __builtin_amdgcn_s_barrier();
      asm volatile("" ::: "memory");
      __builtin_amdgcn_sched_barrier(0);
      issue_x();
      read_x(fx0); read_w(fw0);
      mfmas(fw1, fx1);
      if constexpr (SCHED) interleave(std::integral_constant<int, 2 * C::MI + 2 * C::NJ>{}, std::integral_constant<int, C::XPW>{});
    }
    }
    __builtin_amdgcn_sched_barrier(0);
    TTR_SP_STAMP(1);
    idx += J;
    const bool has_next = idx < xcd_count;
    TTR_SP_NEXT_DELTAS(idx)
    RangeWatch rw;

    if (EM == 0 && (p.dbg_flags & 2)) {
      float sum = 0.f;
#pragma unroll
      for (int j = 0; j < C::NJ; ++j)
#pragma unroll
        for (int i = 0; i < C::MI; ++i) sum += acc[j][i][0] + acc[j][i][1] + acc[j][i][2] + acc[j][i][3];
      if (sum == 1.2345e30f) reinterpret_cast<float*>(p.out ? p.out : (void*)p.out_f32)[0] = sum;
      __builtin_amdgcn_s_waitcnt(0x0F70);
      if (!has_next) break;
      continue;
    }
    if constexpr (EPI == 1) {
      if (p.dbg_flags & 4) {
        float sum = 0.f;
#pragma unroll
        for (int j = 0; j < C::NJ; ++j)
#pragma unroll
          for (int i = 0; i < C::MI; ++i) sum += acc[j][i][0] + acc[j][i][1] + acc[j][i][2] + acc[j][i][3];
        if (sum == 1.2345e30f) reinterpret_cast<float*>(p.out)[0] = sum;
        if (!has_next) break;
        continue;
      }
      typedef __attribute__((ext_vector_type(4))) _Float16 f16x4;
      constexpr int KV = 16384;
      unsigned char* const sQ = smem + C::LDS;
      unsigned char* const sK = sQ + 24576;
      const float osc = p.out_scale;
      const int kR0 = wm * 32 + (((fr >> 2) & 1) << 4) + ((fr >> 3) << 2) + (fr & 3);
      const int kwr = kR0 * 128 + (((wn * 4 + fg) ^ ((kR0 >> 1) & 7)) << 4);
      const int krd = fr * 128 + (((wn * 4 + fg) ^ ((fr >> 1) & 7)) << 4);
      const int qwr = (wm * 2 + (1 - wn)) * 3072 + lane * 16, qrd = (wm * 2 + wn) * 3072 + lane * 16;
      const int vwr = (wm * 32 + fr) * 128 + wn * 64 + fg * 8;
      const float* const bp = p.bias + n0c + wn * 96 + fg * 8;
      f16x8 fq[2][3];
      f16x8 vp[2][2];
      const f16 dn = (f16)(1.f / 2048.f);
      const f16x8 dnv = {dn, dn, dn, dn, dn, dn, dn, dn};
      auto tile_values = [&](int t, int i, float (&v)[8]) {
        const float4 b0 = *reinterpret_cast<const float4*>(bp + t * 32), b1 = *reinterpret_cast<const float4*>(bp + t * 32 + 4);
        const float bv[8] = {b0.x, b0.y, b0.z, b0.w, b1.x, b1.y, b1.z, b1.w};
#pragma unroll
        for (int e = 0; e < 4; ++e) { v[e] = fmaf(acc[2 * t][i][e], osc, bv[e]); v[4 + e] = fmaf(acc[2 * t + 1][i][e], osc, bv[4 + e]); }
      };
      {
        float v0[8], v1[8], keep[8], send[8];
        tile_values(0, 0, v0); tile_values(0, 1, v1);
#pragma unroll
        for (int e = 0; e < 8; ++e) { keep[e] = wn ? v1[e] : v0[e]; send[e] = wn ? v0[e] : v1[e]; }
        split3_x8(keep, fq[0][0], fq[0][1], fq[0][2], rw);
        f16x8 a, b, c;
// ... 267 lines not shown
        if constexpr (EM == 1) {
          gelu_hermite8(v, glut);
          f16x8 a, b;
          split2_x8(v, a, b, rw);
          if (p.out_tiled == 2) {
            const int kb = p.out_ld >> 5;
            f16* o = reinterpret_cast<f16*>(p.out) + ((int64_t)(m >> 4) * (2 * kb) + (n >> 5)) * 512 + ((n >> 3) & 3) * 128 + (m & 15) * 8;
            if (p.store_policy == 1) { __builtin_nontemporal_store(a, reinterpret_cast<f16x8*>(o)); __builtin_nontemporal_store(b, reinterpret_cast<f16x8*>(o + kb * 512)); }
            else { *reinterpret_cast<f16x8*>(o) = a; *reinterpret_cast<f16x8*>(o + kb * 512) = b; }
          } else {
          const int kb = p.out_ld >> 6;
          f16* o = reinterpret_cast<f16*>(p.out) + ((int64_t)(m >> 3) * (2 * kb) + (n >> 6)) * 512 + (m & 7) * 64 + (n & 63);
          *reinterpret_cast<f16x8*>(o) = a; *reinterpret_cast<f16x8*>(o + kb * 512) = b;
          }
          __builtin_amdgcn_sched_barrier(0);
          continue;
        } else if constexpr (EM == 2) {
          sp_store_f32x8(p.out_f32 + (int64_t)m * p.out_f32_ld + n, v);
          continue;
        }
        if (e_act == kActRelu) {
#pragma unroll
          for (int e = 0; e < 8; ++e) v[e] = fmaxf(v[e], 0.f);
        } else if (e_act == kActGelu) {
          if (e_lut) gelu_hermite8(v, glut);
          else {
#pragma unroll
            for (int e = 0; e < 8; ++e) v[e] = gelu_exact(v[e]);
          }
        }
        if (p.dbg_flags & 1) { if (v[0] == 1.2345e30f) reinterpret_cast<float*>(p.out)[0] = v[1]; continue; }
        if (p.out) {
          if (p.out_planes == 3 && p.out_full_cols > 0 && n >= p.out_full_cols) {
            f16x8 a, b, c;
            split3_x8(v, a, b, c, rw);
            f16* o = reinterpret_cast<f16*>(p.out) + (int64_t)m * (3 * (int64_t)p.out_ld) + n;
            *reinterpret_cast<f16x8*>(o) = a; *reinterpret_cast<f16x8*>(o + p.out_ld) = b;
          } else if (p.out_planes && p.out_tiled) {
            const int kb = p.out_tiled == 2 ? p.out_ld >> 5 : p.out_ld >> 6;
            f16* o = p.out_tiled == 2 ? reinterpret_cast<f16*>(p.out) + ((int64_t)(m >> 4) * (p.out_planes * kb) + (n >> 5)) * 512 + ((n >> 3) & 3) * 128 + (m & 15) * 8
                                      : reinterpret_cast<f16*>(p.out) + ((int64_t)(m >> 3) * (p.out_planes * kb) + (n >> 6)) * 512 + (m & 7) * 64 + (n & 63);
            f16x8 a, b, c;
            if (p.out_planes == 3) { split3_x8(v, a, b, c, rw); *reinterpret_cast<f16x8*>(o + 2 * kb * 512) = c; }
            else split2_x8(v, a, b, rw);
            *reinterpret_cast<f16x8*>(o) = a; *reinterpret_cast<f16x8*>(o + kb * 512) = b;
          } else if (p.out_planes) st_split_n(p.out, (int64_t)m, p.out_ld, n, v, p.out_planes, rw);
          else sp_store_f32x8(reinterpret_cast<float*>(p.out) + (int64_t)m * p.out_ld + n, v);
        }
        if (p.out_f32) sp_store_f32x8(p.out_f32 + (int64_t)m * p.out_f32_ld + n, v);
      }
    }
    __builtin_amdgcn_s_waitcnt(0x0F70);
    rw.flush(p.range_flag, p.range_tag);
    if (!has_next) break;
  }
}

#undef TTR_SP_NEXT_DELTAS
#undef TTR_SP_STAMP

static int g_sp_stagger = 0, g_sp_stagger_groups = 2;
void set_gemm_sp_stagger(int v) { g_sp_stagger = v; }
void set_gemm_sp_stagger_groups(int v) { g_sp_stagger_groups = v < 1 ? 1 : v; }

template <int BM, int BN, int WM, int WN, int XST, int WST, int MINB, bool SCHED, int NP = 3, int EPI = 0, int EM = 0, bool KS3 = false, int DBG = 0, bool STAG = false>
static void launch_sp(const ConvParams& p_in, hipStream_t s) {
  using C = SpCfg<BM, BN, WM, WN, XST, WST>;
  constexpr int TABLE = EPI == 1 ? 57344 : 8208;
  ConvParams p = with_range_ctx(p_in);
  p.cu_stagger = g_sp_stagger; p.cu_stagger_groups = g_sp_stagger_groups;
  if ((size_t)(C::LDS + TABLE) * MINB > 160 * 1024) p.gelu_lut = nullptr;
  static PerDeviceOnce once;
  static_assert(EPI == 0 || C::LDS + TABLE <= 160 * 1024, "attention epilogue: rings + images must fit the LDS");
  once.run([&] { TTR_HIP_CHECK(hipFuncSetAttribute((const void*)gemm_sp_kernel<BM, BN, WM, WN, XST, WST, MINB, SCHED, NP, EPI, EM, KS3, DBG, STAG>, hipFuncAttributeMaxDynamicSharedMemorySize, std::min(C::LDS + TABLE, 160 * 1024))); });
  const size_t lds = C::LDS + (EPI == 1 || (p.act == kActGelu && p.gelu_lut) ? TABLE : 0);
  const int tilesM = (p.M + BM - 1) / BM, tilesN = (p.Cout + BN - 1) / BN;
  const int cap = device_cu_count(256) * MINB / 8 * 8;
  const int grid = std::min((tilesM * tilesN + 7) / 8 * 8, std::max(cap, 8));
  hipLaunchKernelGGL((gemm_sp_kernel<BM, BN, WM, WN, XST, WST, MINB, SCHED, NP, EPI, EM, KS3, DBG, STAG>), dim3(grid), dim3(C::NT), lds, s, p);
}

static int g_qkv_attn_dbg = 0;
void set_qkv_attn_dbg(int v) { g_qkv_attn_dbg = v; }
static unsigned long long* g_qkv_attn_stamps = nullptr;
void set_qkv_attn_stamps(unsigned long long* d) { g_qkv_attn_stamps = d; }
static int g_sp_few = 1;
void set_gemm_sp_few(int v) { g_sp_few = v; }
static int g_sp_epi = 3;
static int g_sp_epi_unused = 3;
void set_gemm_sp_epi(int v) { g_sp_epi = v; }
static int g_sp_stag = 0;
void set_gemm_sp_stag(int v) { g_sp_stag = v; }
static int g_sp_dbg = 0;
void set_gemm_sp_dbg(int v) { g_sp_dbg = v; }
static int g_sp_sched = 1;
void set_gemm_sp_sched(int v) { g_sp_sched = v; }

bool gemm_sp_eligible(const ConvParams& p) {
  if (p.up_z) return false;
  if (p.out_tiled && (!p.out_planes || p.out_ld % 64 != 0 || p.out_full_cols)) return false;
  if ((p.out_tiled == 2 || p.x_tiled == 2) && p.M % 16 != 0) return false;
  if ((p.split != 3 && p.split != 4) || p.ks != 1 || p.C1 != 0 || p.out_pool || p.out_relu || p.C0 % 64 != 0 || p.Cout % 8 != 0) return false;
  if (p.split == 3 ? p.C0 < 192 : (p.C0 < 128 || (p.C0 >> 6) % 2 != 0)) return false;
  if (p.resid && (size_t)(p.resid_mod ? p.resid_mod : p.M) * p.resid_ld * 4 >= ((size_t)1 << 31)) return false;
  return (size_t)p.M * p.C0 * (p.split == 3 ? 4 : 6) < ((size_t)1 << 31) && (size_t)p.Cout * p.C0 * 6 < ((size_t)1 << 31);
}

static int g_sp_ks3 = 1;
void set_gemm_sp_ks3(int v) { g_sp_ks3 = v; }
bool gemm_sp_ks3_eligible(const ConvParams& p) {
  if (!g_sp_ks3 || p.split != 3 || p.ks != 3 || p.dil < 1 || p.C1 != 0 || p.out_pool || p.out_relu || p.C0 % 64 != 0 || p.Cout % 8 != 0) return false;
  if (p.x_tiled || p.out_tiled || p.wgt_tiled || p.up_z || p.resid || p.out_full_cols || p.skip) return false;
  if (p.M != p.B * p.H * p.W || p.H >= 32768 || p.W >= 65536) return false;
  return (size_t)p.M * p.C0 * 4 < ((size_t)1 << 31) && (size_t)((p.Cout + 31) / 32 * 32) * 9 * p.C0 * 6 < ((size_t)1 << 31);
}
void launch_gemm_sp_ks3(const ConvParams& p, int cfg, hipStream_t s) {
  if (!gemm_sp_ks3_eligible(p)) throw std::runtime_error("gemm_sp (3x3 taps): shape not supported");
  const int tiles128 = ((p.M + 127) / 128) * ((p.Cout + 127) / 128);
  if (cfg == 2) launch_sp<256, 128, 4, 2, 3, 3, 1, true, 3, 0, 0, true>(p, s);
  else if (g_sp_few && g_sp_ks3 != 3 && tiles128 <= device_cu_count(256)) launch_sp<64, 128, 2, 4, 3, 3, 1, true, 3, 0, 0, true>(p, s);
  else launch_sp<128, 128, 2, 2, 3, 2, 2, true, 3, 0, 0, true>(p, s);
}

void launch_gemm_sp(const ConvParams& p, int cfg, hipStream_t s) {
  if (!gemm_sp_eligible(p)) throw std::runtime_error("gemm_sp: shape not supported");
  const bool sched = g_sp_sched != 0;
  const bool table = p.act == kActGelu && p.gelu_lut;
  const int cus = device_cu_count(256);
  const int tiles128 = ((p.M + 127) / 128) * ((p.Cout + 127) / 128);
  const bool few = cfg == 3 && g_sp_few && 2 * tiles128 <= cus;
  const int tiles96 = ((p.M + 95) / 96) * ((p.Cout + 127) / 128);
  const int rounds128 = (tiles128 + cus - 1) / cus, rounds96 = (tiles96 + cus - 1) / cus;
  const bool mid = cfg == 3 && g_sp_few == 1 && !few && tiles128 <= 4 * cus && rounds96 * 224 < rounds128 * 256 && !(p.act == kActGelu && p.gelu_lut);
  const bool plain = sched && p.dbg_flags == 0;
  const bool em_fc1 = plain && (g_sp_epi & 1) && table && !p.resid && p.out && p.out_planes == 2 && p.out_tiled && !p.out_full_cols && !p.out_f32;
  const bool em_res = plain && (g_sp_epi & (few ? 4 : (p.split == 4 && cfg == 2) ? 2 : 8)) && p.act == kActNone && p.resid && !p.out && p.out_f32;
  const bool lines_fc1 = em_fc1 && (g_sp_epi & 16) && p.out_tiled == 1 && p.M % 16 == 0 && p.Cout % 64 == 0;
  const bool lines_res = plain && (g_sp_epi & 32) && p.act == kActNone && p.resid && !p.out && p.out_f32 && p.M % 16 == 0 && p.Cout % 32 == 0 && !few;
  if (p.split == 4) {
    if (few) { if (em_res) launch_sp<64, 128, 2, 4, 3, 2, 1, true, 4, 0, 2>(p, s); else launch_sp<64, 128, 2, 4, 3, 2, 1, true, 4>(p, s); return; }
    if (mid) { launch_sp<96, 128, 2, 2, 3, 2, 2, true, 4>(p, s); return; }
    if (cfg == 6) launch_sp<128, 256, 2, 4, 3, 2, 1, true, 4>(p, s);
    else if (cfg == 2) { if (lines_res) launch_sp<256, 128, 4, 2, 3, 2, 1, true, 4, 0, 4>(p, s); else if (em_res) launch_sp<256, 128, 4, 2, 3, 2, 1, true, 4, 0, 2>(p, s); else launch_sp<256, 128, 4, 2, 3, 2, 1, true, 4>(p, s); }
    else { if (lines_res) launch_sp<128, 128, 2, 2, 3, 2, 2, true, 4, 0, 4>(p, s); else if (em_res) launch_sp<128, 128, 2, 2, 3, 2, 2, true, 4, 0, 2>(p, s); else launch_sp<128, 128, 2, 2, 3, 2, 2, true, 4>(p, s); }
    return;
  }
  if (few) { if (em_res) launch_sp<64, 128, 2, 4, 3, 3, 1, true, 3, 0, 2>(p, s); else launch_sp<64, 128, 2, 4, 3, 3, 1, true>(p, s); return; }
  if (mid) { launch_sp<96, 128, 2, 2, 3, 2, 2, true>(p, s); return; }
  if (cfg == 6 && em_fc1 && g_sp_dbg) {
    if (g_sp_dbg == 1) launch_sp<128, 256, 2, 4, 3, 3, 1, true, 3, 0, 1, false, 1>(p, s); else if (g_sp_dbg == 4) launch_sp<128, 256, 2, 4, 3, 3, 1, true, 3, 0, 1, false, 4>(p, s); else launch_sp<128, 256, 2, 4, 3, 3, 1, true, 3, 0, 1, false, 8>(p, s);
    return;
  }
  if (cfg != 6 && cfg != 2 && !table && !em_res && sched && g_sp_dbg) {
    if (g_sp_dbg == 1) launch_sp<128, 128, 2, 2, 3, 2, 2, true, 3, 0, 0, false, 1>(p, s); else if (g_sp_dbg == 4) launch_sp<128, 128, 2, 2, 3, 2, 2, true, 3, 0, 0, false, 4>(p, s); else launch_sp<128, 128, 2, 2, 3, 2, 2, true, 3, 0, 0, false, 8>(p, s);
    return;
  }
  if (cfg == 6 && em_fc1 && !lines_fc1 && g_sp_stag) { launch_sp<128, 256, 2, 4, 3, 3, 1, true, 3, 0, 1, false, 0, true>(p, s); return; }
  if (cfg == 6) { if (lines_fc1) launch_sp<128, 256, 2, 4, 3, 3, 1, true, 3, 0, 3>(p, s); else if (em_fc1) launch_sp<128, 256, 2, 4, 3, 3, 1, true, 3, 0, 1>(p, s); else if (sched) launch_sp<128, 256, 2, 4, 3, 3, 1, true>(p, s); else launch_sp<128, 256, 2, 4, 3, 3, 1, false>(p, s); }
  else if (cfg == 2) { if (em_fc1) launch_sp<256, 128, 4, 2, 3, 3, 1, true, 3, 0, 1>(p, s); else if (sched) launch_sp<256, 128, 4, 2, 3, 3, 1, true>(p, s); else launch_sp<256, 128, 4, 2, 3, 3, 1, false>(p, s); }
  else if (table) { if (em_fc1) launch_sp<128, 128, 2, 2, 2, 2, 2, true, 3, 0, 1>(p, s); else if (sched) launch_sp<128, 128, 2, 2, 2, 2, 2, true>(p, s); else launch_sp<128, 128, 2, 2, 2, 2, 2, false>(p, s); }
  else { if (lines_res && mid == false) launch_sp<128, 128, 2, 2, 3, 2, 2, true, 3, 0, 4>(p, s); else if (em_res) launch_sp<128, 128, 2, 2, 3, 2, 2, true, 3, 0, 2>(p, s); else if (sched) launch_sp<128, 128, 2, 2, 3, 2, 2, true>(p, s); else launch_sp<128, 128, 2, 2, 3, 2, 2, false>(p, s); }
}

void launch_qkv_attn_split(const void* x_pairs, const void* w_planes, const float* bias, float inv_scale, void* out_planes, int N, hipStream_t s, const void* w_tiled,
                           int x_tiled, int out_tiled) {
  if (N <= 0) return;
  if (qkv_attn4_enabled()) return launch_qkv_attn4(x_pairs, w_planes, bias, inv_scale, out_planes, N, s, w_tiled, x_tiled, out_tiled);
  if (((uintptr_t)x_pairs | (uintptr_t)w_planes | (uintptr_t)bias | (uintptr_t)out_planes) & 15) throw std::runtime_error("qkv_attn_split: operands must be 16-byte aligned");
  if ((size_t)N * 128 * 384 * 6 >= ((size_t)1 << 31)) throw std::runtime_error("qkv_attn_split: too many crops for 32-bit buffer offsets (the caller groups them)");
  ConvParams p{};
  p.in0 = x_pairs; p.C0 = 384; p.B = 1; p.H = 1; p.W = N * 128; p.ks = 1; p.dil = 1;
  p.wgt = w_planes; p.wgt_tiled = w_tiled; p.bias = bias; p.split = 3; p.out_scale = inv_scale; p.out_planes = 3;
  p.x_tiled = x_tiled; p.out_tiled = out_tiled;
  p.out = out_planes; p.out_ld = 384; p.Cout = 1152; p.M = N * 128; p.act = kActNone;
  p.dbg_flags = g_qkv_attn_dbg; p.dbg = g_qkv_attn_stamps;
  launch_sp<128, 192, 4, 2, 3, 2, 1, true, 3, 1>(p, s);
}

// ... 2 lines not shown
```

tuatara_amd/csrc/kernels.h:

```cpp
#pragma once
#include <stdexcept>
#include "common.h"

namespace ttr {

struct RangeCtx { unsigned* flag = nullptr; unsigned tag = 0; };
RangeCtx& range_ctx();
inline ConvParams with_range_ctx(const ConvParams& p) {
  ConvParams q = p;
  if (!q.range_flag) { q.range_flag = range_ctx().flag; q.range_tag = range_ctx().tag; }
  return q;
}

unsigned* tile_counters(hipStream_t s);

const char* igemm_check(const ConvParams& p);
void launch_igemm(Precision prec, const ConvParams& p, hipStream_t s);
void set_gemm_config(int cfg);
int gemm_config();

const char* gemm2_check(const ConvParams& p);
void launch_gemm2(const ConvParams& p, int cfg, hipStream_t s);
void set_gemm2_split_dbg(int v);
void set_gemm2_split_wreg(int v);
void set_gemm2_split_stream(int v);
void set_gemm2_split_stream4(int v);
bool gemm_sp_eligible(const ConvParams& p);
void set_gemm_sp_sched(int v);
void set_gemm_sp_few(int v);
void set_gemm_sp_epi(int v);
void set_gemm_sp_ks3(int v);
void set_gemm_sp_dbg(int v);
void set_gemm_sp_stag(int v);
void set_gemm_sp_stagger(int v);
void set_gemm_sp_stagger_groups(int v);
void set_qkv_attn_dbg(int v);
void set_qkv_attn_stamps(unsigned long long* dev_buf);
bool gemm_sp_ks3_eligible(const ConvParams& p);
void launch_gemm_sp_ks3(const ConvParams& p, int cfg, hipStream_t s);
void set_gemm_skx_ln_max_rows(int v);
void launch_gemm_sp(const ConvParams& p, int cfg, hipStream_t s);
void set_gemm2_split_cfg(int v);
void set_gemm2_split_few(int v);
void set_gemm2_split_reuse(int v);
void set_gemm2_x_ring3(int v);
const void* gelu_lut_for_current_device();
const void* gelu_hermite_lut_for_current_device();
bool gemm_skx_eligible(const ConvParams& p);
bool gemm_skx_ln_eligible(const ConvParams& p);
void launch_gemm_skx(const ConvParams& p, hipStream_t s);
const char* gemm_sk_check(const ConvParams& p);
void launch_gemm_sk(const ConvParams& p, hipStream_t s);
void set_skinny_max_rows(int m);
void set_mlp_store_nt(int v);
void set_mlp_stamps(unsigned long long* dev_buf);
void launch_dec_cross_attn_mfma(const bf16* q, const bf16* kvmem, bf16* out, int N, int R, hipStream_t s);
void launch_dec_cross_attn_split(const float* q, const float* kvmem, void* out_planes, int N, int R, hipStream_t s);
void set_dec_cross_rows_hsplit(int v);
void set_dec_cross_split(int v);
void set_dec_cross_crop(int v);
void set_dec_cross_mfma(int v);
void set_dec_self_refine(int v);
void set_conv3p_stamps(unsigned long long* dev_buf);
void set_gemm_ws_stamps(unsigned long long* dev_buf);
extern int g_store_policy;
void set_store_policy(int v);
bool conv1u_eligible(const ConvParams& p);
void launch_conv1u(const ConvParams& p, hipStream_t s);
void set_qkv_attn4(int v);
int qkv_attn4_enabled();
void set_qkv_attn4_stamps(unsigned long long* dev_buf);
void launch_qkv_attn4(const void* x_pairs, const void* w_planes, const float* bias, float inv_scale, void* out_planes, int N, hipStream_t s, const void* w_tiled, int x_tiled,
                      int out_tiled);
void set_gemm2_up_resident(int v);
void set_gemm2_up_2d(int v);
bool conv3h_eligible(const ConvParams& p);
void launch_conv3h(const ConvParams& p, hipStream_t s);
void set_conv3h_wgs_per_cu(int v);
void set_conv3h_stamps(unsigned long long* dev_buf);
void set_conv3p_head_persistent(int v);
void set_gemm_ws_dbg_flags(int f);
void set_gemm_ws_lean(int v);
int skinny_max_rows();
// ... 148 lines not shown
```

tuatara_amd/csrc/split.h:

```cpp
#pragma once
#include <hip/hip_runtime.h>

namespace ttr {

typedef _Float16 f16;
typedef __attribute__((ext_vector_type(2))) _Float16 f16x2;
typedef __attribute__((ext_vector_type(2))) float f32x2;
typedef __attribute__((ext_vector_type(8))) _Float16 f16x8;

struct RangeWatch {
  float m = 0.f;
  __device__ __forceinline__ void note(float a, float b) {
#if defined(__HIP_DEVICE_COMPILE__)
    asm("v_max3_f32 %0, %0, |%1|, |%2|" : "+v"(m) : "v"(a), "v"(b));
#else
    m = fmaxf(m, fmaxf(fabsf(a), fabsf(b)));
#endif
  }
  __device__ __forceinline__ void note8(const float (&v)[8]) {
#pragma unroll
    for (int e = 0; e < 8; e += 2) note(v[e], v[e + 1]);
  }
  __device__ __forceinline__ void flush(unsigned* flag, unsigned tag) const {
    if (flag && !(m < 65504.f)) atomicCAS(flag, 0u, tag);
// ... 24 lines not shown
  asm("v_fma_mix_f32 %0, %1, %2, %3 op_sel_hi:[1,0,0]" : "=v"(r) : "v"(h), "s"(c), "v"(x));
  return r;
#else
  return fmaf((float)h[0], c, x);
#endif
}
__device__ __forceinline__ float fma_f16_hi(f16x2 h, float c, float x) {
#if defined(__HIP_DEVICE_COMPILE__)
  float r;
  asm("v_fma_mix_f32 %0, %1, %2, %3 op_sel:[1,0,0] op_sel_hi:[1,0,0]" : "=v"(r) : "v"(h), "s"(c), "v"(x));
  return r;
#else
  return fmaf((float)h[1], c, x);
#endif
}

__device__ __forceinline__ void split3_pair(float a, float b, f16x2& p0, f16x2& p1, f16x2& p2, RangeWatch& rw) {
  rw.note(a, b);
  p0 = __builtin_bit_cast(f16x2, __builtin_amdgcn_cvt_pkrtz(a, b));
  const f32x2 ab = f32x2{a, b} * 2048.f;
  const float ra = fma_f16_lo(p0, -2048.f, ab[0]), rb = fma_f16_hi(p0, -2048.f, ab[1]);
  p1 = __builtin_bit_cast(f16x2, __builtin_amdgcn_cvt_pkrtz(ra, rb));
  const float sa = less_f16_lo(ra, p1), sb = less_f16_hi(rb, p1);
  p2 = f16x2{(f16)sa, (f16)sb};
}
__device__ __forceinline__ void split3_x8(const float (&v)[8], f16x8& o0, f16x8& o1, f16x8& o2, RangeWatch& rw) {
#pragma unroll
  for (int e = 0; e < 8; e += 2) {
    f16x2 a, b, c;
    split3_pair(v[e], v[e + 1], a, b, c, rw);
    o0[e] = a[0]; o0[e + 1] = a[1]; o1[e] = b[0]; o1[e + 1] = b[1]; o2[e] = c[0]; o2[e + 1] = c[1];
  }
}
__device__ __forceinline__ float join3(f16 a, f16 b, f16 c) { return (float)a + ((float)b + (float)c) * (1.f / 2048.f); }

__device__ __forceinline__ void split2_pair(float a, float b, f16x2& p0, f16x2& p1, RangeWatch& rw) {
  rw.note(a, b);
  a = __builtin_amdgcn_fmed3f(a, -65504.f, 65504.f); b = __builtin_amdgcn_fmed3f(b, -65504.f, 65504.f);
  p0 = f16x2{(f16)a, (f16)b};
  const f32x2 ab = f32x2{a, b} * 2048.f;
  const float ra = fma_f16_lo(p0, -2048.f, ab[0]), rb = fma_f16_hi(p0, -2048.f, ab[1]);
  p1 = f16x2{(f16)ra, (f16)rb};
}
__device__ __forceinline__ void split2_x8(const float (&v)[8], f16x8& o0, f16x8& o1, RangeWatch& rw) {
#pragma unroll
  for (int e = 0; e < 8; e += 2) {
    f16x2 a, b;
    split2_pair(v[e], v[e + 1], a, b, rw);
    o0[e] = a[0]; o0[e + 1] = a[1]; o1[e] = b[0]; o1[e + 1] = b[1];
  }
}
__device__ __forceinline__ float join2(f16 a, f16 b) { return (float)a + (float)b * (1.f / 2048.f); }

__device__ __forceinline__ void st_split_n(void* out, int64_t m, int ld, int n, const float (&v)[8], int planes, RangeWatch& rw) {
  if (planes == 3) {
    f16x8 a, b, c;
    split3_x8(v, a, b, c, rw);
    f16* o = reinterpret_cast<f16*>(out) + m * (3 * (int64_t)ld) + n;
    *reinterpret_cast<f16x8*>(o) = a; *reinterpret_cast<f16x8*>(o + ld) = b; *reinterpret_cast<f16x8*>(o + 2 * ld) = c;
  } else if (planes == 2) {
    f16x8 a, b;
    split2_x8(v, a, b, rw);
    f16* o = reinterpret_cast<f16*>(out) + m * (2 * (int64_t)ld) + n;
    *reinterpret_cast<f16x8*>(o) = a; *reinterpret_cast<f16x8*>(o + ld) = b;
  } else {
    float* o = reinterpret_cast<float*>(out) + m * ld + n;
    *reinterpret_cast<float4*>(o) = make_float4(v[0], v[1], v[2], v[3]);
    *reinterpret_cast<float4*>(o + 4) = make_float4(v[4], v[5], v[6], v[7]);
  }
}

__device__ __forceinline__ void st_split_one(void* out, int64_t row, int ld, int c, float v, int planes, RangeWatch& rw) {
  if (planes == 3) {
    f16x2 a, b, d;
    split3_pair(v, 0.f, a, b, d, rw);
    f16* o = reinterpret_cast<f16*>(out) + row * (3 * (int64_t)ld) + c;
    o[0] = a[0]; o[ld] = b[0]; o[2 * ld] = d[0];
  } else {
    reinterpret_cast<float*>(out)[row * ld + c] = v;
  }
}

__host__ __device__ __forceinline__ constexpr int split_xplane(int q) { return q == 3 ? 0 : q; }
__host__ __device__ __forceinline__ constexpr int split_wplane(int q) { return q == 0 ? 0 : q == 3 ? 2 : 1; }

__device__ __forceinline__ void ln384_row8(const float (&v)[8], bool act, const float* gamma8, const float* beta8, float eps, float (&y)[8]) {
  constexpr int D = 384;
  float s = 0.f;
#pragma unroll
  for (int e = 0; e < 8; ++e) s += act ? v[e] : 0.f;
#pragma unroll
  for (int o = 32; o > 0; o >>= 1) s += __shfl_xor(s, o);
  const float mean = s * (1.0f / D);
  float q = 0.f;
#pragma unroll
  for (int e = 0; e < 8; ++e) { const float d = act ? v[e] - mean : 0.f; q = fmaf(d, d, q); }
#pragma unroll
  for (int o = 32; o > 0; o >>= 1) q += __shfl_xor(q, o);
  const float rstd = rsqrtf(fmaf(q, 1.0f / D, eps));
  const float4 g0 = *reinterpret_cast<const float4*>(gamma8), g1 = *reinterpret_cast<const float4*>(gamma8 + 4);
  const float4 b0 = *reinterpret_cast<const float4*>(beta8), b1 = *reinterpret_cast<const float4*>(beta8 + 4);
  const float gg[8] = {g0.x, g0.y, g0.z, g0.w, g1.x, g1.y, g1.z, g1.w}, bb[8] = {b0.x, b0.y, b0.z, b0.w, b1.x, b1.y, b1.z, b1.w};
#pragma unroll
  for (int e = 0; e < 8; ++e) y[e] = fmaf(__fmul_rn(v[e] - mean, rstd), gg[e], bb[e]);
}

// ... 2 lines not shown
```

tuatara_amd/csrc/split_ops.hip:

```cpp
#include <algorithm>

#include "common.h"
#include "kernels.h"
#include "split.h"

namespace ttr {

template <int NPL>
__global__ __launch_bounds__(256) void split_planes_kernel(const float* __restrict__ in, int ld, f16* __restrict__ out, int64_t M, int C, int relu, const int* skip, int skip_n,
                                                          unsigned* range_flag, unsigned range_tag) {
  if (skip && __builtin_nontemporal_load(skip) >= skip_n) return;
  RangeWatch rw;
  const int cv = C >> 3;
  const int64_t total = M * cv;
  for (int64_t i = (int64_t)blockIdx.x * 256 + threadIdx.x; i < total; i += (int64_t)gridDim.x * 256) {
    const int64_t m = i / cv;
    const int c = (int)(i - m * cv) << 3;
    const float* src = in + m * ld + c;
    const float4 a = *reinterpret_cast<const float4*>(src), b = *reinterpret_cast<const float4*>(src + 4);
    float v[8] = {a.x, a.y, a.z, a.w, b.x, b.y, b.z, b.w};
    if (relu) {
#pragma unroll
      for (int e = 0; e < 8; ++e) v[e] = fmaxf(v[e], 0.f);
    }
    st_split_n(out, m, C, c, v, NPL, rw);
  }
  rw.flush(range_flag, range_tag);
}

void launch_split_planes(const float* in, int ld, void* out, int64_t M, int C, int relu, hipStream_t s, int planes, const int* skip, int skip_n) {
  if (M <= 0) return;
  if (C % 8 || ld % 4 || ((uintptr_t)in & 15) || ((uintptr_t)out & 15)) throw std::runtime_error("split_planes: C must be a multiple of 8 and the tensors 16-byte aligned");
  const int64_t total = M * (C >> 3);
  const int grid = (int)std::min<int64_t>((total + 255) / 256, 256 * 32);
  if (planes == 2) hipLaunchKernelGGL(split_planes_kernel<2>, dim3(grid), dim3(256), 0, s, in, ld, (f16*)out, M, C, relu, skip, skip_n, range_ctx().flag, range_ctx().tag);
  else hipLaunchKernelGGL(split_planes_kernel<3>, dim3(grid), dim3(256), 0, s, in, ld, (f16*)out, M, C, relu, skip, skip_n, range_ctx().flag, range_ctx().tag);
}

}

namespace ttr {
namespace {

struct V8 { float v[8]; };
template <int NPL> __device__ __forceinline__ V8 ld_planes(const f16* p, int C) {
  const f16x8 a = *reinterpret_cast<const f16x8*>(p), b = *reinterpret_cast<const f16x8*>(p + C);
  V8 r;
  if constexpr (NPL == 3) {
    const f16x8 c = *reinterpret_cast<const f16x8*>(p + 2 * C);
#pragma unroll
    for (int e = 0; e < 8; ++e) r.v[e] = join3(a[e], b[e], c[e]);
  } else {
#pragma unroll
    for (int e = 0; e < 8; ++e) r.v[e] = join2(a[e], b[e]);
  }
  return r;
}
template <int NPL> __device__ __forceinline__ void st_planes(f16* p, int C, const V8& r, RangeWatch& rw) {
  if constexpr (NPL == 3) {
    f16x8 a, b, c;
    split3_x8(r.v, a, b, c, rw);
    *reinterpret_cast<f16x8*>(p) = a; *reinterpret_cast<f16x8*>(p + C) = b; *reinterpret_cast<f16x8*>(p + 2 * C) = c;
  } else {
    f16x8 a, b;
    split2_x8(r.v, a, b, rw);
    *reinterpret_cast<f16x8*>(p) = a; *reinterpret_cast<f16x8*>(p + C) = b;
  }
}

template <int NPL>
__global__ __launch_bounds__(256) void maxpool3x3s1_planes_kernel(const f16* __restrict__ in, f16* __restrict__ out, int B, int H, int W, int C) {
  const int Cc = C >> 3;
  const int64_t idx = (int64_t)blockIdx.x * 256 + threadIdx.x, total = (int64_t)B * H * W * Cc;
  if (idx >= total) return;
  const int cc = (int)(idx % Cc); int64_t t = idx / Cc;
  const int x = (int)(t % W); t /= W;
  const int y = (int)(t % H); const int b = (int)(t / H);
  V8 m;
#pragma unroll
  for (int e = 0; e < 8; ++e) m.v[e] = -INFINITY;
  for (int dy = -1; dy <= 1; ++dy)
    for (int dx = -1; dx <= 1; ++dx) {
      const int yy = y + dy, xx = x + dx;
      if (yy < 0 || yy >= H || xx < 0 || xx >= W) continue;
      const V8 v = ld_planes<NPL>(in + (((int64_t)b * H + yy) * W + xx) * (NPL * (int64_t)C) + cc * 8, C);
#pragma unroll
      for (int e = 0; e < 8; ++e) m.v[e] = fmaxf(m.v[e], v.v[e]);
    }
  RangeWatch rw;
  st_planes<NPL>(out + (((int64_t)b * H + y) * W + x) * (NPL * (int64_t)C) + cc * 8, C, m, rw);
}

__device__ __forceinline__ float bilerp_s(float v00, float v01, float v10, float v11, float lx0, float lx1, float ly0, float ly1) {
  const float top = fmaf(lx1, v01, lx0 * v00), bot = fmaf(lx1, v11, lx0 * v10);
  return fmaf(ly1, bot, ly0 * top);
}
template <int NPL>
__global__ __launch_bounds__(256) void upsample2x_planes_kernel(const f16* __restrict__ in, f16* __restrict__ out, int B, int H, int W, int C) {
  const int Ho = 2 * H, Wo = 2 * W, Cc = C >> 3;
  const int64_t idx = (int64_t)blockIdx.x * 256 + threadIdx.x, total = (int64_t)B * Ho * Wo * Cc;
  if (idx >= total) return;
  const int cc = (int)(idx % Cc); int64_t t = idx / Cc;
  const int xo = (int)(t % Wo); t /= Wo;
  const int yo = (int)(t % Ho); const int b = (int)(t / Ho);
  const float sy = fmaxf(0.5f * ((float)yo + 0.5f) - 0.5f, 0.f), sx = fmaxf(0.5f * ((float)xo + 0.5f) - 0.5f, 0.f);
  const int y0 = (int)sy, x0 = (int)sx;
  const int y1 = y0 + (y0 < H - 1 ? 1 : 0), x1 = x0 + (x0 < W - 1 ? 1 : 0);
  const float ly1 = sy - (float)y0, ly0 = 1.f - ly1, lx1 = sx - (float)x0, lx0 = 1.f - lx1;
  const f16* base = in + (int64_t)b * H * W * (NPL * (int64_t)C) + cc * 8;
  const int64_t ps = NPL * (int64_t)C;
  const V8 v00 = ld_planes<NPL>(base + ((int64_t)y0 * W + x0) * ps, C), v01 = ld_planes<NPL>(base + ((int64_t)y0 * W + x1) * ps, C);
  const V8 v10 = ld_planes<NPL>(base + ((int64_t)y1 * W + x0) * ps, C), v11 = ld_planes<NPL>(base + ((int64_t)y1 * W + x1) * ps, C);
  V8 o;
#pragma unroll
  for (int e = 0; e < 8; ++e) o.v[e] = bilerp_s(v00.v[e], v01.v[e], v10.v[e], v11.v[e], lx0, lx1, ly0, ly1);
  RangeWatch rw;
  st_planes<NPL>(out + (((int64_t)b * Ho + yo) * Wo + xo) * ps + cc * 8, C, o, rw);
}

template <int NPL, bool FULL>
__global__ __launch_bounds__(256, NPL == 2 ? 4 : 3) void conv1_split_kernel(const uint8_t* __restrict__ canvas, const f16* __restrict__ wgt , const float* __restrict__ bias,
                                                         float out_scale, f16* __restrict__ out , int B, int H, int W, unsigned* range_flag, unsigned range_tag) {
// ... 179 lines not shown
```

tuatara_amd/engine.py:

```python
from __future__ import annotations

import collections.abc
import ctypes as C
import os
import sys
from typing import List, Optional, Sequence

import numpy as np

_LIBPATH = os.environ.get("TUATARA_LIB") or os.path.join(os.path.dirname(os.path.abspath(__file__)), "lib", "libtuatara_hip.so")
_lib = None

PREC_BF16, PREC_F32, PREC_F16X4 = 0, 1, 2
CROP_BOUNDING, CROP_RECTIFIED = 0, 1
ORIENT_OFF, ORIENT_FLIP, ORIENT_QUARTER = 0, 1, 2


class Config(C.Structure):
    _fields_ = [("precision", C.c_int), ("device", C.c_int), ("canvas_size", C.c_int), ("mag_ratio", C.c_float),
                ("text_threshold", C.c_float), ("link_threshold", C.c_float), ("low_text", C.c_float), ("min_area", C.c_int),
                ("strict_crops", C.c_int), ("max_components", C.c_int), ("verbose", C.c_int), ("crop_mode", C.c_int),
                ("orient", C.c_int), ("orient_page", C.c_int), ("lines", C.c_int), ("chars", C.c_int), ("blocks", C.c_int),
                ("mixed_batches", C.c_int)]

# ... 74 lines not shown
    ("ttr_result_block_order", _PI, [_VP]),
    ("ttr_result_block_first", _PI, [_VP]),
    ("ttr_result_block_bboxes", _PF, [_VP]),
    ("ttr_result_block_text", _I, [_VP, _I, C.c_char_p, C.c_size_t]),
    ("ttr_result_page_text_blocks", _I, [_VP, C.c_char_p, C.c_size_t]),
    ("ttr_results_gather_blocks", _I, [C.POINTER(_VP), _I, _PI, _PI, _PI, _PI, _PI, _PI, _PI, _PF]),
    ("ttr_blocks_from_quads", _I, [_PF, _I, _PI, _PI, _PI, _PI, _PI, _PI, _PI]),
    ("ttr_group_blocks", _I, [_VP, _PF, _PI, _I, _PI, _PI, _PI, _PI, _PI, _PI, _PI]),
    ("ttr_result_free", None, [_VP]),
    ("ttr_result_bboxes", _PF, [_VP]),
    ("ttr_result_ids_all", _PI, [_VP]),
    ("ttr_result_texts", _I, [_VP, C.c_char_p, C.c_size_t]),
    ("ttr_results_gather", _I, [C.POINTER(_VP), _I, _PI, _PF, _PI, C.c_char_p, C.c_size_t, C.POINTER(C.c_size_t)]),
    ("ttr_results_gather_conf", _I, [C.POINTER(_VP), _I, _PF, _PF]),
    ("ttr_confidence_from_probs", _I, [_PI, _PF, _I, _PF, C.POINTER(C.c_int), _PF]),
    ("ttr_logits_confidence", _I, [_VP, _PF, _I, _PI, _PF, _PF]),
    ("ttr_charset_mask", _I, [C.c_char_p, C.c_char_p, C.POINTER(C.c_uint32)]),
    ("ttr_engine_set_charset", _I, [_VP, C.c_char_p, C.c_char_p]),
    ("ttr_engine_get_charset", _I, [_VP, C.POINTER(C.c_uint32)]),
    ("ttr_logits_confidence_masked", _I, [_VP, _PF, _I, C.POINTER(C.c_uint32), _PI, _PF, _PF]),
    ("ttr_region_from_rect", _I, [_I, _I, _I, _I, _PF]),
    ("ttr_region_geometry", _I, [_PF, _I, _I, C.POINTER(C.c_int64), _PF, C.POINTER(C.c_int)]),
    ("ttr_regions_to_data_dev", _I, [_VP, C.POINTER(Page), _I, C.POINTER(Region), _I, C.POINTER(C.c_uint32), _I, C.POINTER(_VP)]),
    ("ttr_image_regions_to_data", _I, [_VP, _PU8, _I, _I, _I, C.POINTER(Region), _I, C.POINTER(C.c_uint32), _I, C.POINTER(_VP)]),
    ("ttr_result_sets", _PI, [_VP]),
    ("ttr_pack_regions", _I, [_VP, _PU8, _I, _I, _I, _PF, _I, _PU8]),
    ("ttr_parseq_logits_sets", _I, [_VP, _PU8, _I, C.POINTER(C.c_uint32), _I, _PI, _PF, _PF, _PI]),
    ("ttr_logits_confidence_sets", _I, [_VP, _PF, _I, C.POINTER(C.c_uint32), _I, _PI, _PI, _PF, _PF]),
    ("ttr_craft_heatmap", _I, [_VP, _PU8, _I, _I, _PF]),
    ("ttr_ccl_boxes", _I, [_VP, _PF, _I, _I, _PF, _I, _PI]),
    ("ttr_resize_canvas", _I, [_VP, _PU8, _I, _I, _I, _PU8, C.c_size_t, _PI, _PI, _PF]),
    ("ttr_pack_crops", _I, [_VP, _PU8, _I, _I, _I, _PF, _I, _F, _PU8, _PF]),
    ("ttr_pack_crops_rectified", _I, [_VP, _PU8, _I, _I, _I, _PF, _I, _F, _PU8, _PF]),
    ("ttr_pack_crops_oriented", _I, [_VP, _PU8, _I, _I, _I, _PF, _I, _F, _I, _I, _PU8, _PF]),
    ("ttr_parseq_logits", _I, [_VP, _PU8, _I, _PF, _PF, _PI]),
    ("ttr_decode_ids", _I, [_PI, _I, C.c_char_p]),
    ("ttr_engine_set_tuning", _I, [_VP, C.c_char_p, _I]),
    ("ttr_dbg_conv", _I, [_VP, _PF, _I, _PF, _I, _I, _I, _I, _I, _I, _I, _I, _PF, _PF, _I, _I, _PF]),
    ("ttr_dbg_min_area_rect", _I, [_PF, _I, _PF]),
    ("ttr_dbg_tcp_share", _I, [_I, _I, C.c_char_p, _I, _VP, C.c_size_t]),
    ("ttr_dbg_component_rect", _I, [_I, _I, _I, _I, _I, _PI, _I, _I, _PF]),
    ("ttr_dbg_box_geometry", _I, [_PF, _F, _PF, _PI, _PF]),
    ("ttr_dbg_deskew", _I, [_PF, _PF, C.POINTER(C.c_double), C.POINTER(C.c_int64)]),
    ("ttr_dbg_orient_quad", _I, [_PF, _I, _I, _I, _I, _PF, C.POINTER(C.c_int64)]),
    ("ttr_dev_alloc", _VP, [C.c_size_t]),
    ("ttr_dev_free", None, [_VP]),
    ("ttr_dev_upload", _I, [_VP, _VP, C.c_size_t]),
    ("ttr_dev_download", _I, [_VP, _VP, C.c_size_t]),
    ("ttr_dev_sync", _I, [_VP]),
    ("ttr_last_stage_ms", _I, [_VP, _PF]),
    ("ttr_set_profiling", _I, [_VP, _I]),
    ("ttr_dbg_conv_pool", _I, [_VP, _PF, _I, _I, _I, _I, _I, _PF, _PF, _I, _I, _I, _PF, _PF]),
    ("ttr_dbg_split_gemm", _I, [_VP, _PF, _I, _I, _PF, _PF, _I, _I, _I, _I, _PF, _I, _PF]),
    ("ttr_dbg_craft_taps", _I, [_VP, _PU8, _I, _I, _I, _PF]),
    ("ttr_dbg_craft_tap_count", _I, [_VP]),
    ("ttr_dbg_craft_tap_info", _I, [_VP, _I, C.c_char_p, C.c_size_t, _PI]),
    ("ttr_dbg_craft_tap_read", _I, [_VP, _I, _PF]),
    ("ttr_set_gemm_config", None, [_I]),
    ("ttr_set_decoder_mode", None, [_I]),
    ("ttr_set_tuning", _I, [C.c_char_p, _I]),
    ("ttr_last_host_us", None, [_VP, _PF]),
    ("ttr_dbg_attn_enc", _I, [_VP, _PF, _I, _PF]),
    ("ttr_dbg_cross_attn", _I, [_VP, _PF, _PF, _I, _I, _PF]),
    ("ttr_dbg_qkv_attn", _I, [_VP, _PF, _I, _PF, _PF, _PF]),
    ("ttr_dbg_mlp", _I, [_VP, _PF, _I, _PF, _PF, C.c_float, _PF, _PF, _PF, _PF, _PF, _PF, _PF, _PF, _PF, _PF, _PF]),
    ("ttr_dbg_dec_stamps", _I, [C.POINTER(C.c_ulonglong)]),
    ("ttr_dbg_dec_stamps_ext", _I, [C.POINTER(C.c_ulonglong), _I]),
    ("ttr_bench_conv", _I, [_VP, _I, _I, _I, _I, _I, _I, _I, _I, _I, _I, _I, _PF]),
    ("ttr_get_profile", _I, [_VP, C.POINTER(C.c_double), C.POINTER(C.c_double), C.POINTER(C.c_longlong)]),
    ("ttr_get_profile_kinds", _I, [_VP, C.c_char_p, C.c_size_t]),
    ("ttr_comm_unique_id", _I, [_VP]),
    ("ttr_comm_create", _VP, [_VP, _I, _I, _VP]),
    ("ttr_comm_create_tcp", _VP, [_VP, _I, _I, C.c_char_p, _I]),
    ("ttr_comm_create_socket", _VP, [_VP, _I, _I, C.c_char_p, _I]),
    ("ttr_comm_transport", C.c_char_p, [_VP]),
    ("ttr_comm_describe", _I, [_VP, C.c_char_p, C.c_size_t]),
    ("ttr_comm_destroy", None, [_VP]),
    ("ttr_comm_rank", _I, [_VP]),
    ("ttr_comm_world", _I, [_VP]),
    ("ttr_engine_attach_comm", _I, [_VP, _VP]),
    ("ttr_last_gathered", _I, [_VP, C.POINTER(C.c_int), C.POINTER(C.c_int), _PI, C.c_size_t, _PI, C.c_size_t, C.POINTER(C.c_size_t)]),
    ("ttr_last_gathered_conf", _I, [_VP, _PF, C.c_size_t, _PF, C.c_size_t]),
    ("ttr_comm_allgather_host", _I, [_VP, _VP, C.c_size_t, _VP]),
    ("ttr_gather_layout", _I, [_PI, _I, _I, C.POINTER(C.c_int), _PI, C.POINTER(C.c_int64)]),
    ("ttr_pages_to_data_dev_sharded", _I, [_VP, _VP, _I, _I, _I, C.POINTER(_VP)]),
]


def lib_path() -> str:
    return _LIBPATH


def load():
    global _lib
    if _lib is None:
        if not os.path.exists(_LIBPATH):
            raise RuntimeError(f"{_LIBPATH} is missing: run `python -m tuatara_amd.build` (or __graft_entry__.build()) first")
        if "torch" not in sys.modules and os.environ.get("TUATARA_PRELOAD_TORCH", "1") != "0":
            try:
                import torch
            except ImportError:
                pass
        lib = C.CDLL(_LIBPATH)
        for name, res, args in SYMBOLS:
            fn = getattr(lib, name)
            fn.restype = res
            fn.argtypes = args
        _lib = lib
    return _lib


def _u8(a):
    return a.ctypes.data_as(_PU8)


def _f(a):
    return a.ctypes.data_as(_PF)


def _i(a):
    return a.ctypes.data_as(_PI)


class EngineError(RuntimeError):
    pass


def decode_ids(ids: Sequence[int]) -> str:
    a = np.ascontiguousarray(ids, dtype=np.int32)
    buf = C.create_string_buffer(len(a) + 2)
    load().ttr_decode_ids(_i(a), len(a), buf)
    return buf.value.decode("latin1")


def min_area_rect(points) -> np.ndarray:
    pts = np.ascontiguousarray(points, dtype=np.float32).reshape(-1, 2)
    out = np.zeros(5, np.float32)
    load().ttr_dbg_min_area_rect(_f(pts), len(pts), _f(out))
    return out


def component_rect(area: int, x0: int, y0: int, x1: int, y1: int, rows: np.ndarray, H: int, W: int):
    rows = np.ascontiguousarray(rows, dtype=np.int32)
    out = np.zeros(5, np.float32)
    ok = load().ttr_dbg_component_rect(area, x0, y0, x1, y1, _i(rows), H, W, _f(out))
    return out if ok == 1 else None


def box_geometry(rect5, ratio: float):
    r = np.ascontiguousarray(rect5, dtype=np.float32)
    adj, xywh, bbox = np.zeros(5, np.float32), np.zeros(4, np.int32), np.zeros(4, np.float32)
    load().ttr_dbg_box_geometry(_f(r), C.c_float(ratio), _f(adj), _i(xywh), _f(bbox))
    return adj, tuple(int(v) for v in xywh), [float(v) for v in bbox]


def deskew(rect5):
    r = np.ascontiguousarray(rect5, dtype=np.float32)
# ... 798 lines not shown
            so = np.ascontiguousarray(set_of, dtype=np.int32).ravel()
            if len(so) != n:
                raise ValueError("set_of holds one entry per row")
            sp, ns, _keep = _sets_arg(sets)
            self._check(self.lib.ttr_logits_confidence_sets(self.h, _f(logits), n, sp, ns, _i(so), _i(ids), _f(prob), _f(conf)))
        elif mask is None:
            self._check(self.lib.ttr_logits_confidence(self.h, _f(logits), n, _i(ids), _f(prob), _f(conf)))
        else:
            m = (C.c_uint32 * 3)(*[int(v) for v in np.asarray(mask).ravel()[:3]])
            self._check(self.lib.ttr_logits_confidence_masked(self.h, _f(logits), n, m, _i(ids), _f(prob), _f(conf)))
        return ids, prob, conf

    def dbg_conv_pool(self, x0: np.ndarray, w: np.ndarray, bias: Optional[np.ndarray], ks: int, act: int = 0, pool_relu: bool = False,
                      want_full: bool = True):
        x0 = np.ascontiguousarray(x0, dtype=np.float32)
        B, H, W_, C0 = x0.shape
        w = np.ascontiguousarray(w, dtype=np.float32)
        Cout = w.shape[0]
        full = np.zeros((B, H, W_, Cout), np.float32) if want_full else None
        pool = np.zeros((B, H // 2, W_ // 2, Cout), np.float32)
        b = np.ascontiguousarray(bias, dtype=np.float32) if bias is not None else None
        self._check(self.lib.ttr_dbg_conv_pool(self.h, _f(x0), C0, B, H, W_, ks, _f(w), _f(b) if b is not None else None, Cout, act,
                                               int(pool_relu), _f(full) if want_full else None, _f(pool)))
        return full, pool

    def dbg_conv(self, x0: np.ndarray, w: np.ndarray, bias: Optional[np.ndarray], ks: int, dil: int = 1, act: int = 0,
                 x1: Optional[np.ndarray] = None, relu0: bool = False, relu1: bool = False) -> np.ndarray:
        x0 = np.ascontiguousarray(x0, dtype=np.float32)
        B, H, W_, C0 = x0.shape
        C1 = 0
        if x1 is not None:
            x1 = np.ascontiguousarray(x1, dtype=np.float32)
            C1 = x1.shape[-1]
        w = np.ascontiguousarray(w, dtype=np.float32)
        Cout = w.shape[0]
        out = np.zeros((B, H, W_, Cout), np.float32)
        b = np.ascontiguousarray(bias, dtype=np.float32) if bias is not None else None
        self._check(self.lib.ttr_dbg_conv(self.h, _f(x0), C0, _f(x1) if x1 is not None else None, C1, int(relu0), int(relu1), B, H, W_, ks, dil,
                                          _f(w), _f(b) if b is not None else None, Cout, act, _f(out)))
        return out

    def dbg_split_gemm(self, x: np.ndarray, w: np.ndarray, bias: Optional[np.ndarray] = None, np_products: int = 3, act: int = 0, out_planes: int = 0,
                       resid: Optional[np.ndarray] = None, cfg: int = 0) -> np.ndarray:
        x = np.ascontiguousarray(x, dtype=np.float32); w = np.ascontiguousarray(w, dtype=np.float32)
        M, K = x.shape
        N = w.shape[0]
        out = np.zeros((M, N), np.float32)
        b = np.ascontiguousarray(bias, dtype=np.float32) if bias is not None else None
        r = np.ascontiguousarray(resid, dtype=np.float32) if resid is not None else None
        self._check(self.lib.ttr_dbg_split_gemm(self.h, _f(x), M, K, _f(w), _f(b) if b is not None else None, N, np_products, act, out_planes,
                                                _f(r) if r is not None else None, cfg, _f(out)))
        return out


def gather_layout(counts: np.ndarray):
    counts = np.ascontiguousarray(counts, dtype=np.int32)
    world, pages = counts.shape
    cap = C.c_int()
    total = np.zeros(world, np.int32)
    first = np.zeros(world * pages + 1, np.int64)
    if load().ttr_gather_layout(_i(counts), world, pages, C.byref(cap), _i(total), first.ctypes.data_as(C.POINTER(C.c_int64))) != 0:
        raise EngineError(load().ttr_last_error().decode())
    return cap.value, total, first


class Comm:

    def __init__(self, engine: "Engine", rank: int, world: int, addr: str = "127.0.0.1", port: int = 29617, unique_id: Optional[bytes] = None,
                 transport: str = "rccl"):
        self.eng, self.lib = engine, engine.lib
        if transport == "socket":
            self.h = self.lib.ttr_comm_create_socket(engine.h, rank, world, addr.encode(), port)
        elif unique_id is not None:
            buf = C.create_string_buffer(unique_id, 256)
            self.h = self.lib.ttr_comm_create(engine.h, rank, world, buf)
        else:
            self.h = self.lib.ttr_comm_create_tcp(engine.h, rank, world, addr.encode(), port)
        if not self.h:
            raise EngineError(self.lib.ttr_last_error().decode())
        self.rank, self.world = rank, world

    @staticmethod
    def unique_id() -> bytes:
        buf = C.create_string_buffer(256)
        if load().ttr_comm_unique_id(buf) != 0:
            raise EngineError(load().ttr_last_error().decode())
        return buf.raw

    def attach(self, on: bool = True):
        if self.lib.ttr_engine_attach_comm(self.eng.h, self.h if on else None) != 0:
            raise EngineError(self.lib.ttr_last_error().decode())

    def allgather_host(self, mine: np.ndarray) -> np.ndarray:
        mine = np.ascontiguousarray(mine)
        out = np.zeros((self.world,) + mine.shape, mine.dtype)
        if self.lib.ttr_comm_allgather_host(self.h, mine.ctypes.data_as(C.c_void_p), mine.nbytes, out.ctypes.data_as(C.c_void_p)) != 0:
            raise EngineError(self.lib.ttr_last_error().decode())
        return out

    def barrier(self):
        self.allgather_host(np.zeros(1, np.int32))

    def describe(self) -> dict:
        import json
        buf = C.create_string_buffer(512)
        if self.lib.ttr_comm_describe(self.h, buf, len(buf)) < 0:
# ... 39 lines not shown
```

Before: 423.3.

## Fold encoder LayerNorm into split-GEMM row-panel epilogue and regroup encoder chunks

Adds a PANEL mode to the split-precision GEMM kernel. When one workgroup owns a full 384-wide row panel, it computes the following LayerNorm and writes the f16 planes directly, so the separate norm1, norm2 and final-norm launches and their fp32 re-reads can be skipped. The fold is gated by a new `enc_ln_fold` tuning knob that defaults to off, plus an occupancy heuristic. Separately, encoder chunking is rebuilt so chunk sizes are multiples of twice the CU count, with buffer sizing derived from the actual plane counts; this regrouping runs by default. A debug entry point for checking the fold against the unfused LayerNorm is also added.

New measurement: 420.8. No clear change (-0.6%).

```diff
diff --git a/include/tuatara_hip_debug.h b/include/tuatara_hip_debug.h
--- a/include/tuatara_hip_debug.h
+++ b/include/tuatara_hip_debug.h
@@ -12,6 +12,8 @@
 
 int ttr_dbg_split_gemm(ttr_engine* e, const float* x, int M, int K, const float* w, const float* bias, int N, int np, int act, int out_planes,
                        const float* resid, int cfg, float* out);
+int ttr_dbg_ln_fold(ttr_engine* e, const float* x, int M, int K, const float* w, const float* bias, const float* resid, int np, const float* gamma,
+                    const float* beta, float eps, int planes, int tiled, float* rows, uint16_t* folded, uint16_t* ref);
 int ttr_dbg_conv_pool(ttr_engine* e, const float* in0, int C0, int B, int H, int W, int ks, const float* wgt, const float* bias,
                       int Cout, int act, int pool_relu, float* out_full, float* out_pool);
 int ttr_dbg_craft_taps(ttr_engine* e, const uint8_t* canvas, int B, int H, int W, float* heat_out);
diff --git a/tuatara_amd/csrc/capi_debug.cpp b/tuatara_amd/csrc/capi_debug.cpp
--- a/tuatara_amd/csrc/capi_debug.cpp
+++ b/tuatara_amd/csrc/capi_debug.cpp
@@ -95,6 +95,45 @@
       if (out_planes == 3) lo += f16_to_f32(row[2 * N + n]);
       out[(size_t)m * N + n] = (float)(v + lo / 2048.0);
     }
+  return 0;
+  TTR_GUARD_END(-1)
+}
+
+int ttr_dbg_ln_fold(ttr_engine* e, const float* x, int M, int K, const float* w, const float* bias, const float* resid, int np, const float* gamma,
+                    const float* beta, float eps, int planes, int tiled, float* rows, uint16_t* folded, uint16_t* ref) {
+  TTR_GUARD_BEGIN
+  Engine& E = *e->e;
+  EngineScope lk(E);
+  if (E.prec != kSplit) throw std::runtime_error("ttr_dbg_ln_fold: f16x4 engines only");
+  if (np != 3 && np != 4) throw std::runtime_error("ttr_dbg_ln_fold: np must be 3 or 4");
+  const int ipl = np == 3 ? 2 : 3, N = 384;
+  const size_t pbytes = (size_t)((M + 255) / 256 * 256) * N * planes * 2;
+  DevBuf dx, dxp, dout, dres, dg, db, dfold, dref;
+  Linear L;
+  auto up = [&](DevBuf& d, const float* h, size_t n) { d.ensure(n * 4); TTR_HIP_CHECK(hipMemcpy(d.p, h, n * 4, hipMemcpyHostToDevice)); };
+  up(dx, x, (size_t)M * K); up(dres, resid, (size_t)M * N); up(dg, gamma, N); up(db, beta, N);
+  dxp.ensure((size_t)M * K * 2 * ipl);
+  launch_split_planes(dx.as<float>(), K, dxp.p, M, K, 0, E.stream, ipl);
+  E.upload_linear(L, w, N, K, bias, N, K, nullptr, false);
+  if (!L.ws.p) throw std::runtime_error("ttr_dbg_ln_fold: the layer has no weight planes");
+  dout.ensure((size_t)M * N * 4); dfold.ensure(pbytes); dref.ensure(pbytes);
+  TTR_HIP_CHECK(hipMemsetAsync(dfold.p, 0xCD, pbytes, E.stream)); TTR_HIP_CHECK(hipMemsetAsync(dref.p, 0xCD, pbytes, E.stream));
+  ConvParams p{};
+  p.in0 = dxp.p; p.C0 = K; p.B = 1; p.H = 1; p.W = M; p.ks = 1; p.dil = 1;
+  if (E.tn.sp_tiled_w) E.tile_planes(L);
+  p.wgt = L.ws.p; p.bias = L.b.as<float>(); p.split = np; p.out_scale = L.inv_scale;
+  p.wgt_tiled = E.tn.sp_tiled_w ? L.wst.p : nullptr;
+  p.out_f32 = dout.as<float>(); p.out_f32_ld = N; p.resid = dres.as<float>(); p.resid_ld = N;
+  p.Cout = N; p.M = M; p.act = kActNone;
+  p.ln_out = dfold.p; p.ln_fold_gamma = dg.as<float>(); p.ln_fold_beta = db.as<float>(); p.ln_fold_eps = eps; p.ln_planes = planes; p.ln_tiled = tiled;
+  if (!gemm_sp_ln_fold_eligible(p)) throw std::runtime_error("ttr_dbg_ln_fold: shape not supported");
+  if (const char* err = gemm2_check(p)) throw std::runtime_error(err);
+  launch_gemm2(p, 0, E.stream);
+  launch_layernorm_planes(dout.as<float>(), N, dg.as<float>(), db.as<float>(), eps, dref.p, M, E.stream, planes, nullptr, 0, tiled);
+  TTR_HIP_CHECK(hipMemcpyAsync(rows, dout.p, (size_t)M * N * 4, hipMemcpyDeviceToHost, E.stream));
+  TTR_HIP_CHECK(hipMemcpyAsync(folded, dfold.p, pbytes, hipMemcpyDeviceToHost, E.stream));
+  TTR_HIP_CHECK(hipMemcpyAsync(ref, dref.p, pbytes, hipMemcpyDeviceToHost, E.stream));
+  TTR_HIP_CHECK(hipStreamSynchronize(E.stream));
   return 0;
   TTR_GUARD_END(-1)
 }
@@ -376,6 +415,7 @@
   else if (k == "gsp_sched") set_gemm_sp_sched(value);
   else if (k == "gsp_few") set_gemm_sp_few(value);
   else if (k == "gsp_epi") set_gemm_sp_epi(value);
+  else if (k == "gsp_fold_em") set_gemm_sp_fold_em(value);
   else if (k == "gsp_ks3") set_gemm_sp_ks3(value);
   else if (k == "gsp_stagger") set_gemm_sp_stagger(value);
   else if (k == "gsp_dbg") set_gemm_sp_dbg(value);
diff --git a/tuatara_amd/csrc/common.h b/tuatara_amd/csrc/common.h
--- a/tuatara_amd/csrc/common.h
+++ b/tuatara_amd/csrc/common.h
@@ -71,6 +71,7 @@
   unsigned* range_flag; unsigned range_tag;
   int cu_stagger, cu_stagger_groups;
   unsigned* tile_ctr;
+  void* ln_out; const float* ln_fold_gamma; const float* ln_fold_beta; float ln_fold_eps; int ln_planes, ln_tiled; unsigned ln_range_tag;
 };
 
 __device__ __forceinline__ float gelu_exact(float x) { return 0.5f * x * (1.0f + erff(x * 0.70710678118654752440f)); }
diff --git a/tuatara_amd/csrc/engine.h b/tuatara_amd/csrc/engine.h
--- a/tuatara_amd/csrc/engine.h
+++ b/tuatara_amd/csrc/engine.h
@@ -60,6 +60,7 @@
   int sp_tiled_w = 1;
   int ar_host_check = 10;
   int enc_chunk = 0;
+  int enc_ln_fold = 0;
   int enc_ln_pairs = 1;
   int dec_planes = 1;
   int qkv_kv_pairs = 1;
@@ -88,6 +89,7 @@
   bool set(const std::string& k, int value) {
     if (k == "decoder_mode") decoder_mode = value;
     else if (k == "enc_chunk") enc_chunk = value;
+    else if (k == "enc_ln_fold") enc_ln_fold = value;
     else if (k == "range_guard") range_guard = value;
     else if (k == "recog_overlap") recog_overlap = value;
     else if (k == "craft_lanes") craft_lanes = value == 2 ? 2 : 1;
@@ -505,9 +507,10 @@
     if (craft_tap_on && p) craft_taps.push_back(CraftTap{layer, role, kind, p, B, H, W, C, ld, form});
   }
 
+  struct LnFold { std::string name; float eps; void* out; int planes, tiled; };
   void sgemm(const Linear& L, const void* in_planes, int M, void* out, int out_ld, int act, int out_planes,
              float* out_f32 = nullptr, int out_f32_ld = 0, const float* resid = nullptr, int resid_ld = 0, int np = 4, int resid_mod = 0, int out_full_cols = 0,
-             const char* kind = nullptr, int x_tiled = 0, int out_tiled = 0);
+             const char* kind = nullptr, int x_tiled = 0, int out_tiled = 0, const LnFold* ln = nullptr);
   void ln_gemm(const float* x, const std::string& ln_name, float eps, void* scratch, const Linear& L, int M, void* out, int out_ld, int act,
                float* out_f32 = nullptr, int out_f32_ld = 0);
   void gemm(const Linear& L, const void* in, int M, void* out, int out_ld, int act, float* out_f32 = nullptr, int out_f32_ld = 0,
diff --git a/tuatara_amd/csrc/engine_parseq.cpp b/tuatara_amd/csrc/engine_parseq.cpp
--- a/tuatara_amd/csrc/engine_parseq.cpp
+++ b/tuatara_amd/csrc/engine_parseq.cpp
@@ -6,10 +6,16 @@
 
 void Engine::sgemm(const Linear& L, const void* in_planes, int M, void* out, int out_ld, int act, int out_planes,
            float* out_f32, int out_f32_ld, const float* resid, int resid_ld, int np, int resid_mod, int out_full_cols,
-           const char* kind, int x_tiled, int out_tiled) {
+           const char* kind, int x_tiled, int out_tiled, const LnFold* ln) {
   if (!L.ws.p) throw std::runtime_error("split GEMM: the layer has no weight planes");
+  ConvParams p{};
+  if (ln) {
+    range_tag("parseq." + ln->name);
+    p.ln_range_tag = range_ctx().tag;
+    p.ln_out = ln->out; p.ln_fold_gamma = pqf.at(ln->name + ".weight").as<float>(); p.ln_fold_beta = pqf.at(ln->name + ".bias").as<float>(); p.ln_fold_eps = ln->eps;
+    p.ln_planes = ln->planes; p.ln_tiled = ln->tiled;
+  }
   range_tag("parseq." + range_scope + (kind ? kind : "linear"));
-  ConvParams p{};
   p.out_full_cols = out_full_cols;
   p.in0 = in_planes; p.C0 = L.k; p.B = 1; p.H = 1; p.W = M; p.ks = 1; p.dil = 1;
   p.wgt = L.ws.p; p.bias = L.b.as<float>(); p.split = np; p.out_scale = L.inv_scale; p.out_planes = out_planes == 1 ? 3 : out_planes;
@@ -19,7 +25,8 @@
   p.out = out; p.out_ld = out_ld; p.out_f32 = out_f32; p.out_f32_ld = out_f32_ld; p.resid = resid; p.resid_ld = resid_ld; p.resid_mod = resid_mod;
   p.Cout = L.cout_valid ? L.cout_valid : L.cout; p.M = M; p.act = act;
   p.skip = cur_skip; p.skip_n = cur_skip_n;
-  const bool skinny = tn.skinny_split && np == 4 && M <= tn.skinny_max_rows && !x_tiled && !out_tiled && gemm_skx_eligible(p);
+  if (ln && !gemm_sp_ln_fold_eligible(p)) throw std::runtime_error("split GEMM: this layer cannot take the following LayerNorm (gemm_sp.hip, ConvParams::ln_out)");
+  const bool skinny = !ln && tn.skinny_split && np == 4 && M <= tn.skinny_max_rows && !x_tiled && !out_tiled && gemm_skx_eligible(p);
   if (!skinny) { if (const char* e = gemm2_check(p)) throw std::runtime_error(e); }
   if (skinny) {
     timed(kind ? kind : "split linear (triples, skinny)", 2.0 * M * p.Cout * L.k, 2.0 * M * p.Cout * L.k * np, [&] { launch_gemm_skx(p, stream); });
@@ -152,24 +159,46 @@
   gemm(pq.at("patch"), patches, M, nullptr, 0, kActNone, x, E, pqf.at("encoder.pos_embed").as<float>(), E, 128);
   const bool enc_split = prec == kSplit && tn.split_gemm && tn.split_planes;
   if (enc_split) {
-    int CHS = std::max(1, std::min(N, (int)((((size_t)1 << 31) - 1) / ((size_t)128 * 1536 * 6))));
+    const int lnpl = tn.enc_ln_pairs ? 2 : 3;
+    const int hpl = tn.enc_fc2_pairs ? 2 : 3;
+    const bool qkv_attn = tn.qkv_attn_split && lnpl == 2;
+    const size_t big_row = std::max((size_t)1536 * hpl * 2, qkv_attn ? (size_t)0 : (size_t)3 * E * 6);
+    int CHS = std::max(1, std::min(N, (int)((((size_t)1 << 31) - 1) / ((size_t)128 * std::max(big_row, (size_t)E * 6)))));
     if (tn.enc_chunk > 0) CHS = std::min(CHS, tn.enc_chunk);
-    if (N > CHS) { const int groups = (N + CHS - 1) / CHS; CHS = (N + groups - 1) / groups; }
+    const int round = std::max(2 * device_cu_count(256) / 8 * 8, 8);
+    std::vector<int> groups;
+    if (N <= CHS && (N < round || N % round == 0)) groups.push_back(N);
+    else if (CHS >= round) {
+      const int big = CHS / round * round;
+      int left = N;
+      while (left >= round) { const int n = std::min(big, left / round * round); groups.push_back(n); left -= n; }
+      if (left) groups.push_back(left);
+    } else {
+      const int ng = (N + CHS - 1) / CHS, per = (N + ng - 1) / ng;
+      for (int c0 = 0; c0 < N; c0 += per) groups.push_back(std::min(per, N - c0));
+    }
+    const int gmax = *std::max_element(groups.begin(), groups.end());
     void* lnp = (pq_ws[11].ensure((size_t)M * E * 6), pq_ws[11].p);
-    void* bigp = (pq_ws[12].ensure((size_t)std::min(N, CHS) * 128 * 1536 * 6), pq_ws[12].p);
-    void* attp = (pq_ws[13].ensure((size_t)std::min(N, CHS) * 128 * E * 6), pq_ws[13].p);
+    void* bigp = (pq_ws[12].ensure((size_t)gmax * 128 * big_row), pq_ws[12].p);
+    void* attp = (pq_ws[13].ensure((size_t)gmax * 128 * E * 6), pq_ws[13].p);
     auto lnp_at = [&](int c0) { return (char*)lnp + (size_t)c0 * 128 * E * 6; };
-    const int lnpl = tn.enc_ln_pairs ? 2 : 3;
-    const int xt = tn.sp_tiled_x && tn.qkv_attn_split && lnpl == 2 && tn.enc_fc2_pairs && std::min(CHS, N) * 128 > tn.skinny_max_rows ? 1 : 0;
-    for (int c0 = 0; c0 < N; c0 += CHS) {
-      const int nc = std::min(CHS, N - c0), Mc = nc * 128;
+    const int xt = tn.sp_tiled_x && tn.qkv_attn_split && lnpl == 2 && tn.enc_fc2_pairs && gmax * 128 > tn.skinny_max_rows ? 1 : 0;
+    int c0 = 0;
+    for (const int nc : groups) {
+      const int Mc = nc * 128;
       float* xc = x + (size_t)c0 * 128 * E;
+      const bool fold = tn.enc_ln_fold == 2 || (tn.enc_ln_fold == 1 && gemm_sp_ln_fold_fills(Mc, 4) && gemm_sp_ln_fold_fills(Mc, hpl + 1));
+      auto ln_launch = [&](const std::string& name, int planes, int tiled) {
+        range_tag("parseq." + name);
+        timed(planes == 2 ? "enc.layernorm_planes_kernel<2>" : "enc.layernorm_planes_kernel<3>", 0, 0, [&] {
+          launch_layernorm_planes(xc, E, pqf.at(name + ".weight").as<float>(), pqf.at(name + ".bias").as<float>(), 1e-6f, lnp_at(c0), Mc, stream, planes, nullptr, 0, tiled);
+        });
+      };
       for (int l = 0; l < 12; ++l) {
         const std::string p = "encoder.blocks." + std::to_string(l) + ".";
         range_scope = p;
-        range_tag("parseq." + p + "norm1");
-        launch_layernorm_planes(xc, E, pqf.at(p + "norm1.weight").as<float>(), pqf.at(p + "norm1.bias").as<float>(), 1e-6f, lnp_at(c0), Mc, stream, lnpl, nullptr, 0, xt);
-        if (tn.qkv_attn_split && lnpl == 2) {
+        if (l == 0 || !fold) ln_launch(p + "norm1", lnpl, xt);
+        if (qkv_attn) {
           const Linear& L = pq.at(p + "qkv_hm");
           range_tag("parseq." + p + "attn (qkv + attention)");
           const double qa = 2.0 * Mc * 3 * E * E, aa = 2.0 * 2 * nc * 6 * 128.0 * 128 * 64;
@@ -179,17 +208,17 @@
         sgemm(pq.at(p + "qkv"), lnp_at(c0), Mc, bigp, 3 * E, kActNone, 1, nullptr, 0, nullptr, 0, lnpl + 1, 0, tn.qkv_kv_pairs ? E : 0, "enc.qkv");
         range_tag("parseq." + p + "attn.qkv"), launch_attn_enc_split(bigp, attp, nc, stream);
         }
-        sgemm(pq.at(p + "proj"), attp, Mc, nullptr, 0, kActNone, 0, xc, E, xc, E, 4, 0, 0, "enc.proj", xt, 0);
-        range_tag("parseq." + p + "norm2");
-        launch_layernorm_planes(xc, E, pqf.at(p + "norm2.weight").as<float>(), pqf.at(p + "norm2.bias").as<float>(), 1e-6f, lnp_at(c0), Mc, stream, lnpl, nullptr, 0, xt);
-        const int hpl = tn.enc_fc2_pairs ? 2 : 3;
+        const LnFold f2{p + "norm2", 1e-6f, lnp_at(c0), lnpl, xt};
+        sgemm(pq.at(p + "proj"), attp, Mc, nullptr, 0, kActNone, 0, xc, E, xc, E, 4, 0, 0, "enc.proj", xt, 0, fold ? &f2 : nullptr);
+        if (!fold) ln_launch(p + "norm2", lnpl, xt);
         const int hx = xt && tn.sp_hidden16 && hpl == 2 ? 2 : xt;
         sgemm(pq.at(p + "fc1"), lnp_at(c0), Mc, bigp, 4 * E, kActGelu, hpl, nullptr, 0, nullptr, 0, lnpl + 1, 0, 0, "enc.fc1 + GELU", xt, hx);
-        sgemm(pq.at(p + "fc2"), bigp, Mc, nullptr, 0, kActNone, 0, xc, E, xc, E, hpl + 1, 0, 0, "enc.fc2", hx, 0);
+        const LnFold f1 = l < 11 ? LnFold{"encoder.blocks." + std::to_string(l + 1) + ".norm1", 1e-6f, lnp_at(c0), lnpl, xt} : LnFold{"encoder.norm", 1e-6f, lnp_at(c0), 3, 0};
+        sgemm(pq.at(p + "fc2"), bigp, Mc, nullptr, 0, kActNone, 0, xc, E, xc, E, hpl + 1, 0, 0, "enc.fc2", hx, 0, fold ? &f1 : nullptr);
       }
       range_scope.clear();
-      range_tag("parseq.encoder.norm");
-      launch_layernorm_planes(xc, E, pqf.at("encoder.norm.weight").as<float>(), pqf.at("encoder.norm.bias").as<float>(), 1e-6f, lnp_at(c0), Mc, stream);
+      if (!fold) ln_launch("encoder.norm", 3, 0);
+      c0 += nc;
     }
   }
   const bool mlp_fused = prec == kBF16 && gemm_config() >= 0 && (tn.mlp_fused == 2 || (tn.mlp_fused == 1 && M >= tn.mlp_min_rows));
diff --git a/tuatara_amd/csrc/gemm2.hip b/tuatara_amd/csrc/gemm2.hip
--- a/tuatara_amd/csrc/gemm2.hip
+++ b/tuatara_amd/csrc/gemm2.hip
@@ -643,6 +643,7 @@
   if (p.split == 3 && p.ks == 3 && (cfg == 2 || cfg == 3) && g_split_stream && gemm_sp_ks3_eligible(p))
     return launch_gemm_sp_ks3(p, cfg, s);
   if (p.x_tiled || p.out_tiled) throw std::runtime_error("gemm2: tiled planes are gemm_sp.hip's (this shape did not qualify for it)");
+  if (p.ln_out) throw std::runtime_error("gemm2: the LayerNorm behind a row panel is gemm_sp.hip's (this shape did not qualify for it)");
   if (p.split && cfg == 3 && g_split_few && (int64_t)((p.M + 127) / 128) * ((p.Cout + 127) / 128) <= num_cus()) cfg = 5;
   if (p.split) {
     const bool ru = g_split_reuse != 0 || p.split == 3;
diff --git a/tuatara_amd/csrc/gemm_sp.hip b/tuatara_amd/csrc/gemm_sp.hip
--- a/tuatara_amd/csrc/gemm_sp.hip
+++ b/tuatara_amd/csrc/gemm_sp.hip
@@ -17,6 +17,59 @@
 static __device__ __forceinline__ void sp_store_f32x8(float* o, const float (&v)[8]) {
   __builtin_nontemporal_store(f32x4{v[0], v[1], v[2], v[3]}, reinterpret_cast<f32x4*>(o));
   __builtin_nontemporal_store(f32x4{v[4], v[5], v[6], v[7]}, reinterpret_cast<f32x4*>(o + 4));
+}
+
+template <int BM, int NW>
+__device__ __attribute__((noinline)) void sp_ln_panel(const float* rows, int ld, int M, int m0, f16* lnout, const float* gamma, const float* beta, float eps, int planes, int tiled,
+                                                     unsigned* range_flag, unsigned range_tag) {
+  constexpr int D = 384, LNG = 4, RPW = BM / NW;
+  constexpr unsigned OOB = 0x80000000u;
+  static_assert(RPW % (2 * LNG) == 0, "rows per wave: whole pairs of groups");
+  __builtin_amdgcn_s_barrier();
+  asm volatile("" ::: "memory");
+  const int lane = threadIdx.x & 63, wave = __builtin_amdgcn_readfirstlane(threadIdx.x >> 6);
+  const __amdgpu_buffer_rsrc_t rso = sp_rsrc(rows, (unsigned)((size_t)M * ld * 4));
+  const bool lact = lane < 48;
+  const int lc = (lact ? lane : 0) * 8;
+  RangeWatch rwl;
+  auto ln_load = [&](int g, f32x4 (&b)[LNG][2]) {
+#pragma unroll
+    for (int r = 0; r < LNG; ++r) {
+      const int row = m0 + (g * LNG + r) * NW + wave;
+      const unsigned ro = row < M ? ((unsigned)row * (unsigned)ld + (unsigned)lc) * 4u : OOB;
+      b[r][0] = __builtin_bit_cast(f32x4, __builtin_amdgcn_raw_buffer_load_b128(rso, ro, 0, 16));
+      b[r][1] = __builtin_bit_cast(f32x4, __builtin_amdgcn_raw_buffer_load_b128(rso, ro, 16, 16));
+    }
+  };
+  auto ln_rows = [&](int g, const f32x4 (&b)[LNG][2]) {
+#pragma unroll
+    for (int r = 0; r < LNG; ++r) {
+      const int row = m0 + (g * LNG + r) * NW + wave;
+      if (row >= M) continue;
+      const float v[8] = {b[r][0][0], b[r][0][1], b[r][0][2], b[r][0][3], b[r][1][0], b[r][1][1], b[r][1][2], b[r][1][3]};
+      V8 o;
+      ln384_row8(v, lact, gamma + lc, beta + lc, eps, o.v);
+      if (!lact) continue;
+      if (planes == 2) {
+        if (tiled) st_planes<2>(lnout + ((int64_t)(row >> 3) * (2 * 6) + (lc >> 6)) * 512 + (row & 7) * 64 + (lc & 63), 6 * 512, o, rwl);
+        else st_planes<2>(lnout + (int64_t)row * (2 * D) + lc, D, o, rwl);
+      } else {
+        if (tiled) st_planes<3>(lnout + ((int64_t)(row >> 3) * (3 * 6) + (lc >> 6)) * 512 + (row & 7) * 64 + (lc & 63), 6 * 512, o, rwl);
+        else st_planes<3>(lnout + (int64_t)row * (3 * D) + lc, D, o, rwl);
+      }
+    }
+  };
+  f32x4 la[LNG][2], lb[LNG][2];
+  ln_load(0, la);
+#pragma unroll 1
+  for (int g = 0; g < RPW / LNG; g += 2) {
+    ln_load(g + 1, lb);
+    ln_rows(g, la);
+    if (g + 2 < RPW / LNG) ln_load(g + 2, la);
+    ln_rows(g + 1, lb);
+  }
+  __builtin_amdgcn_s_waitcnt(0x0F70);
+  rwl.flush(range_flag, range_tag);
 }
 
 template <int BM, int BN, int WM, int WN, int XST, int WST>
@@ -31,7 +84,7 @@
   static_assert((BM / 8) % NW == 0 && (BN / 8) % NW == 0 && TN % 32 == 0 && TM % 16 == 0, "tile shape");
 };
 
-template <int BM, int BN, int WM, int WN, int XST, int WST, int MINB, bool SCHED, int NP, int EPI = 0, int EM = 0, bool KS3 = false, int DBG = 0, bool STAG = false>
+template <int BM, int BN, int WM, int WN, int XST, int WST, int MINB, bool SCHED, int NP, int EPI = 0, int EM = 0, bool KS3 = false, int DBG = 0, bool STAG = false, bool PANEL = false>
 __global__ __launch_bounds__(WM * WN * 64, MINB) void gemm_sp_kernel(ConvParams p) {
   using C = SpCfg<BM, BN, WM, WN, XST, WST>;
   static_assert(NP == 3 || (NP == 4 && XST == 3 && WST == 2), "pairs, or triples on rings 3 + 2");
@@ -46,13 +99,14 @@
   static_assert(EM == 0 || EPI == 0, "fixed epilogue cases are the plain epilogue's");
   static_assert(!KS3 || (NP == 3 && EPI == 0), "3x3 taps: the pairs loop");
   static_assert(!STAG || (NP == 3 && WM * WN == 8 && SCHED), "staggered halves: the pairs loop on eight waves");
+  static_assert(!PANEL || (EPI == 0 && !KS3 && DBG == 0 && (EM == 0 || EM == 2)), "panel schedule: the plain epilogue's residual case");
   float2* const glut = reinterpret_cast<float2*>(smem + C::LDS);
   if (EM == 1 || EM == 3 || (EM == 0 && p.act == kActGelu && p.gelu_lut)) {
     for (int i = tid; i < 512; i += C::NT) reinterpret_cast<uint4*>(glut)[i] = reinterpret_cast<const uint4*>(p.gelu_lut)[i];
   }
 
   const int tilesM = (p.M + BM - 1) / BM, tilesN = (p.Cout + BN - 1) / BN;
-  const int T = tilesM * tilesN;
+  const int T = PANEL ? tilesM : tilesM * tilesN;
   const int xcd = blockIdx.x & 7, J = gridDim.x >> 3;
   int xcd_first, xcd_count;
   {
@@ -60,8 +114,21 @@
     xcd_first = xcd < r ? xcd * (q + 1) : r * (q + 1) + (xcd - r) * q;
     xcd_count = q + (xcd < r ? 1 : 0);
   }
-  int idx = blockIdx.x >> 3;
-  if (idx >= xcd_count) return;
+  const int wg = blockIdx.x >> 3;
+  if (wg >= xcd_count) return;
+  int idx = PANEL ? 0 : wg;
+  const int STEP = PANEL ? 1 : J;
+  auto tile_at = [&](int li, bool& live, int& m0, int& n0) {
+    if constexpr (PANEL) {
+      const int pi = li / tilesN, pl = wg + pi * J;
+      live = pl < xcd_count;
+      m0 = (xcd_first + pl) * BM; n0 = (li - pi * tilesN) * BN;
+    } else {
+      live = li < xcd_count;
+      const int tile = xcd_first + li, tm = tile / tilesN;
+      m0 = tm * BM; n0 = (tile - tm * tilesN) * BN;
+    }
+  };
   if (p.cu_stagger > 0) {
     const unsigned long long wait = (unsigned long long)((blockIdx.x >> 3) % p.cu_stagger_groups) * (unsigned)p.cu_stagger / (unsigned)p.cu_stagger_groups;
     const unsigned long long t0 = __builtin_amdgcn_s_memrealtime();
@@ -82,8 +149,8 @@
   unsigned char* const wring = smem + XST * C::XBYTES;
 
   auto tile_offsets = [&](int li, unsigned (&xo)[C::XPW], unsigned (&wo)[C::WPW]) {
-    const bool live = li < xcd_count;
-    const int tile = xcd_first + li, tm = tile / tilesN, m0 = tm * BM, n0 = (tile - tm * tilesN) * BN;
+    bool live; int m0, n0;
+    tile_at(li, live, m0, n0);
 #pragma unroll
     for (int i = 0; i < C::XPW; ++i) {
       const int row = (i * C::NW + wave) * 8 + (lane >> 3);
@@ -184,7 +251,7 @@
   {                                                                              \
     unsigned xa_[C::XPW], wa_[C::WPW], xb_[C::XPW], wb_[C::WPW];                 \
     tile_offsets((LI), xa_, wa_);                                                \
-    tile_offsets((LI) + J, xb_, wb_);                                            \
+    tile_offsets((LI) + STEP, xb_, wb_);                                         \
     _Pragma("unroll") for (int i = 0; i < C::XPW; ++i) xdl[i] = xb_[i] - xa_[i]; \
     _Pragma("unroll") for (int j = 0; j < C::WPW; ++j) wdl[j] = wb_[j] - wa_[j]; \
   }
@@ -259,8 +326,8 @@
     for (int j = 0; j < C::NJ; ++j)
 #pragma unroll
       for (int i = 0; i < C::MI; ++i) acc[j][i] = f32x4{0.f, 0.f, 0.f, 0.f};
-    const int ctile = xcd_first + idx;
-    const int m0c = (ctile / tilesN) * BM, n0c = (ctile % tilesN) * BN;
+    int m0c, n0c;
+    { bool live_c; tile_at(idx, live_c, m0c, n0c); }
 
     auto mfmas = [&](const f16x8 (&fw)[2][C::NJ], const f16x8 (&fx)[2][C::MI]) {
 #pragma unroll
@@ -408,8 +475,9 @@
     }
     __builtin_amdgcn_sched_barrier(0);
     TTR_SP_STAMP(1);
-    idx += J;
-    const bool has_next = idx < xcd_count;
+    idx += STEP;
+    bool has_next;
+    { int m0n, n0n; tile_at(idx, has_next, m0n, n0n); }
     TTR_SP_NEXT_DELTAS(idx)
     RangeWatch rw;
 
@@ -783,6 +851,9 @@
     }
     __builtin_amdgcn_s_waitcnt(0x0F70);
     rw.flush(p.range_flag, p.range_tag);
+    if constexpr (PANEL) {
+      if (n0c + BN >= p.Cout) sp_ln_panel<BM, C::NW>(p.out_f32, p.out_f32_ld, p.M, m0c, reinterpret_cast<f16*>(p.ln_out), p.ln_fold_gamma, p.ln_fold_beta, p.ln_fold_eps, p.ln_planes, p.ln_tiled, p.range_flag, p.ln_range_tag);
+    }
     if (!has_next) break;
   }
 }
@@ -794,7 +865,7 @@
 void set_gemm_sp_stagger(int v) { g_sp_stagger = v; }
 void set_gemm_sp_stagger_groups(int v) { g_sp_stagger_groups = v < 1 ? 1 : v; }
 
-template <int BM, int BN, int WM, int WN, int XST, int WST, int MINB, bool SCHED, int NP = 3, int EPI = 0, int EM = 0, bool KS3 = false, int DBG = 0, bool STAG = false>
+template <int BM, int BN, int WM, int WN, int XST, int WST, int MINB, bool SCHED, int NP = 3, int EPI = 0, int EM = 0, bool KS3 = false, int DBG = 0, bool STAG = false, bool PANEL = false>
 static void launch_sp(const ConvParams& p_in, hipStream_t s) {
   using C = SpCfg<BM, BN, WM, WN, XST, WST>;
   constexpr int TABLE = EPI == 1 ? 57344 : 8208;
@@ -803,12 +874,12 @@
   if ((size_t)(C::LDS + TABLE) * MINB > 160 * 1024) p.gelu_lut = nullptr;
   static PerDeviceOnce once;
   static_assert(EPI == 0 || C::LDS + TABLE <= 160 * 1024, "attention epilogue: rings + images must fit the LDS");
-  once.run([&] { TTR_HIP_CHECK(hipFuncSetAttribute((const void*)gemm_sp_kernel<BM, BN, WM, WN, XST, WST, MINB, SCHED, NP, EPI, EM, KS3, DBG, STAG>, hipFuncAttributeMaxDynamicSharedMemorySize, std::min(C::LDS + TABLE, 160 * 1024))); });
+  once.run([&] { TTR_HIP_CHECK(hipFuncSetAttribute((const void*)gemm_sp_kernel<BM, BN, WM, WN, XST, WST, MINB, SCHED, NP, EPI, EM, KS3, DBG, STAG, PANEL>, hipFuncAttributeMaxDynamicSharedMemorySize, std::min(C::LDS + TABLE, 160 * 1024))); });
   const size_t lds = C::LDS + (EPI == 1 || (p.act == kActGelu && p.gelu_lut) ? TABLE : 0);
   const int tilesM = (p.M + BM - 1) / BM, tilesN = (p.Cout + BN - 1) / BN;
   const int cap = device_cu_count(256) * MINB / 8 * 8;
-  const int grid = std::min((tilesM * tilesN + 7) / 8 * 8, std::max(cap, 8));
-  hipLaunchKernelGGL((gemm_sp_kernel<BM, BN, WM, WN, XST, WST, MINB, SCHED, NP, EPI, EM, KS3, DBG, STAG>), dim3(grid), dim3(C::NT), lds, s, p);
+  const int grid = std::min(((PANEL ? tilesM : tilesM * tilesN) + 7) / 8 * 8, std::max(cap, 8));
+  hipLaunchKernelGGL((gemm_sp_kernel<BM, BN, WM, WN, XST, WST, MINB, SCHED, NP, EPI, EM, KS3, DBG, STAG, PANEL>), dim3(grid), dim3(C::NT), lds, s, p);
 }
 
 static int g_qkv_attn_dbg = 0;
@@ -853,8 +924,30 @@
   else launch_sp<128, 128, 2, 2, 3, 2, 2, true, 3, 0, 0, true>(p, s);
 }
 
+bool gemm_sp_ln_fold_eligible(const ConvParams& p) {
+  if (!gemm_sp_eligible(p) || !p.ln_out || !p.ln_fold_gamma || !p.ln_fold_beta) return false;
+  if (p.Cout != 384 || p.act != kActNone || !p.resid || p.out || !p.out_f32 || p.dbg_flags || p.out_f32_ld % 4 != 0) return false;
+  if ((p.ln_planes != 2 && p.ln_planes != 3) || (p.ln_tiled && p.M % 8 != 0)) return false;
+  if (((uintptr_t)p.out_f32 | (uintptr_t)p.ln_out | (uintptr_t)p.ln_fold_gamma | (uintptr_t)p.ln_fold_beta) & 15) return false;
+  return (size_t)p.M * p.out_f32_ld * 4 < ((size_t)1 << 31);
+}
+bool gemm_sp_ln_fold_fills(int M, int split) {
+  const int bm = split == 4 ? 256 : 128, G = std::max(device_cu_count(256) * (split == 4 ? 1 : 2) / 8 * 8, 8);
+  const int64_t P = (M + bm - 1) / bm, T = 3 * P;
+  return (P + G - 1) / G * 3 <= (T + G - 1) / G;
+}
+static int g_sp_fold_em = 0;
+void set_gemm_sp_fold_em(int v) { g_sp_fold_em = v; }
+static void launch_gemm_sp_ln_fold(const ConvParams& p, hipStream_t s) {
+  if (!gemm_sp_ln_fold_eligible(p) || !g_sp_sched) throw std::runtime_error("gemm_sp: this layer cannot take the LayerNorm behind its row panels (ConvParams::ln_out)");
+  if (p.split == 4) launch_sp<256, 128, 4, 2, 3, 2, 1, true, 4, 0, 2, false, 0, false, true>(p, s);
+  else if (g_sp_fold_em == 2) launch_sp<128, 128, 2, 2, 3, 2, 2, true, 3, 0, 2, false, 0, false, true>(p, s);
+  else launch_sp<128, 128, 2, 2, 3, 2, 2, true, 3, 0, 0, false, 0, false, true>(p, s);
+}
+
 void launch_gemm_sp(const ConvParams& p, int cfg, hipStream_t s) {
   if (!gemm_sp_eligible(p)) throw std::runtime_error("gemm_sp: shape not supported");
+  if (p.ln_out) return launch_gemm_sp_ln_fold(p, s);
   const bool sched = g_sp_sched != 0;
   const bool table = p.act == kActGelu && p.gelu_lut;
   const int cus = device_cu_count(256);
diff --git a/tuatara_amd/csrc/kernels.h b/tuatara_amd/csrc/kernels.h
--- a/tuatara_amd/csrc/kernels.h
+++ b/tuatara_amd/csrc/kernels.h
@@ -26,9 +26,12 @@
 void set_gemm2_split_stream(int v);
 void set_gemm2_split_stream4(int v);
 bool gemm_sp_eligible(const ConvParams& p);
+bool gemm_sp_ln_fold_eligible(const ConvParams& p);
+bool gemm_sp_ln_fold_fills(int M, int split);
 void set_gemm_sp_sched(int v);
 void set_gemm_sp_few(int v);
 void set_gemm_sp_epi(int v);
+void set_gemm_sp_fold_em(int v);
 void set_gemm_sp_ks3(int v);
 void set_gemm_sp_dbg(int v);
 void set_gemm_sp_stag(int v);
diff --git a/tuatara_amd/csrc/split.h b/tuatara_amd/csrc/split.h
--- a/tuatara_amd/csrc/split.h
+++ b/tuatara_amd/csrc/split.h
@@ -100,6 +100,19 @@
 }
 __device__ __forceinline__ float join2(f16 a, f16 b) { return (float)a + (float)b * (1.f / 2048.f); }
 
+struct V8 { float v[8]; };
+template <int NPL> __device__ __forceinline__ void st_planes(f16* p, int C, const V8& r, RangeWatch& rw) {
+  if constexpr (NPL == 3) {
+    f16x8 a, b, c;
+    split3_x8(r.v, a, b, c, rw);
+    *reinterpret_cast<f16x8*>(p) = a; *reinterpret_cast<f16x8*>(p + C) = b; *reinterpret_cast<f16x8*>(p + 2 * C) = c;
+  } else {
+    f16x8 a, b;
+    split2_x8(r.v, a, b, rw);
+    *reinterpret_cast<f16x8*>(p) = a; *reinterpret_cast<f16x8*>(p + C) = b;
+  }
+}
+
 __device__ __forceinline__ void st_split_n(void* out, int64_t m, int ld, int n, const float (&v)[8], int planes, RangeWatch& rw) {
   if (planes == 3) {
     f16x8 a, b, c;
diff --git a/tuatara_amd/csrc/split_ops.hip b/tuatara_amd/csrc/split_ops.hip
--- a/tuatara_amd/csrc/split_ops.hip
+++ b/tuatara_amd/csrc/split_ops.hip
@@ -42,7 +42,6 @@
 namespace ttr {
 namespace {
 
-struct V8 { float v[8]; };
 template <int NPL> __device__ __forceinline__ V8 ld_planes(const f16* p, int C) {
   const f16x8 a = *reinterpret_cast<const f16x8*>(p), b = *reinterpret_cast<const f16x8*>(p + C);
   V8 r;
@@ -56,18 +55,6 @@
   }
   return r;
 }
-template <int NPL> __device__ __forceinline__ void st_planes(f16* p, int C, const V8& r, RangeWatch& rw) {
-  if constexpr (NPL == 3) {
-    f16x8 a, b, c;
-    split3_x8(r.v, a, b, c, rw);
-    *reinterpret_cast<f16x8*>(p) = a; *reinterpret_cast<f16x8*>(p + C) = b; *reinterpret_cast<f16x8*>(p + 2 * C) = c;
-  } else {
-    f16x8 a, b;
-    split2_x8(r.v, a, b, rw);
-    *reinterpret_cast<f16x8*>(p) = a; *reinterpret_cast<f16x8*>(p + C) = b;
-  }
-}
-
 template <int NPL>
 __global__ __launch_bounds__(256) void maxpool3x3s1_planes_kernel(const f16* __restrict__ in, f16* __restrict__ out, int B, int H, int W, int C) {
   const int Cc = C >> 3;
diff --git a/tuatara_amd/engine.py b/tuatara_amd/engine.py
--- a/tuatara_amd/engine.py
+++ b/tuatara_amd/engine.py
@@ -150,6 +150,7 @@
     ("ttr_set_profiling", _I, [_VP, _I]),
     ("ttr_dbg_conv_pool", _I, [_VP, _PF, _I, _I, _I, _I, _I, _PF, _PF, _I, _I, _I, _PF, _PF]),
     ("ttr_dbg_split_gemm", _I, [_VP, _PF, _I, _I, _PF, _PF, _I, _I, _I, _I, _PF, _I, _PF]),
+    ("ttr_dbg_ln_fold", _I, [_VP, _PF, _I, _I, _PF, _PF, _PF, _I, _PF, _PF, C.c_float, _I, _I, _PF, C.POINTER(C.c_uint16), C.POINTER(C.c_uint16)]),
     ("ttr_dbg_craft_taps", _I, [_VP, _PU8, _I, _I, _I, _PF]),
     ("ttr_dbg_craft_tap_count", _I, [_VP]),
     ("ttr_dbg_craft_tap_info", _I, [_VP, _I, C.c_char_p, C.c_size_t, _PI]),
@@ -201,6 +202,8 @@
                 pass
         lib = C.CDLL(_LIBPATH)
         for name, res, args in SYMBOLS:
+            if os.environ.get("TUATARA_LIB") and not hasattr(lib, name):
+                continue
             fn = getattr(lib, name)
             fn.restype = res
             fn.argtypes = args
@@ -1105,6 +1108,21 @@
                                                 _f(r) if r is not None else None, cfg, _f(out)))
         return out
 
+    def dbg_ln_fold(self, x: np.ndarray, w: np.ndarray, bias: np.ndarray, resid: np.ndarray, gamma: np.ndarray, beta: np.ndarray, np_products: int = 3,
+                    eps: float = 1e-6, planes: int = 2, tiled: bool = False):
+        x = np.ascontiguousarray(x, dtype=np.float32); w = np.ascontiguousarray(w, dtype=np.float32)
+        M, K = x.shape
+        assert w.shape == (384, K) and resid.shape == (M, 384)
+        b, r = np.ascontiguousarray(bias, dtype=np.float32), np.ascontiguousarray(resid, dtype=np.float32)
+        g, be = np.ascontiguousarray(gamma, dtype=np.float32), np.ascontiguousarray(beta, dtype=np.float32)
+        rows = np.zeros((M, 384), np.float32)
+        pad = (M + 255) // 256 * 256
+        folded, ref = np.zeros((pad, planes * 384), np.uint16), np.zeros((pad, planes * 384), np.uint16)
+        u16 = C.POINTER(C.c_uint16)
+        self._check(self.lib.ttr_dbg_ln_fold(self.h, _f(x), M, K, _f(w), _f(b), _f(r), np_products, _f(g), _f(be), float(eps), planes, int(bool(tiled)),
+                                             _f(rows), folded.ctypes.data_as(u16), ref.ctypes.data_as(u16)))
+        return rows, folded, ref
+
 
 def gather_layout(counts: np.ndarray):
     counts = np.ascontiguousarray(counts, dtype=np.int32)
```
